# NNU-GISA/MetricSfM

Hardware: AMD Instinct MI355X
Metric: BA iterations/sec (higher is better)
Workload: dtype f64; 1 GPU; BASELINE config 3: 500 cameras / 200000 points / 1200000 observations, dense-Schur LM, Huber(1); reduced_system_order=3003, parallelism=points sharded over 1 rank(s), camera block all-reduced, collective=none (1 rank), successful_steps=2789, unsuccessful_steps=0

## Files before the change

### include/msfm.h

```cpp
#ifndef MSFM_H_
#define MSFM_H_

#include <stddef.h>
#include <stdint.h>

#ifdef __cplusplus
extern "C" {
#endif

#define MSFM_VERSION 100

#define MSFM_OK 0
#define MSFM_E_INVAL (-1)
#define MSFM_E_NOMEM (-2)
#define MSFM_E_DEVICE (-3)
#define MSFM_E_NUMERIC (-4)

typedef struct msfm_ctx msfm_ctx;

int msfm_version(void);
int msfm_ctx_create(int device, msfm_ctx** out);
void msfm_ctx_destroy(msfm_ctx* ctx);
const char* msfm_last_error(const msfm_ctx* ctx);
void* msfm_ctx_stream(msfm_ctx* ctx);
// ... 65 lines not shown

typedef struct msfm_ba_options {
  int max_num_iterations;
  int num_threads;
  int progress_to_stdout;
  double huber_delta;
  double function_tolerance;
  double gradient_tolerance;
  double parameter_tolerance;
  double initial_trust_region_radius;
  double max_trust_region_radius;
  double min_trust_region_radius;
  double min_relative_decrease;
  double min_lm_diagonal;
  double max_lm_diagonal;
  int max_num_consecutive_invalid_steps;
  int jacobi_scaling;
} msfm_ba_options;
void msfm_ba_options_default(msfm_ba_options* opt);

#define MSFM_BA_CONVERGENCE_FUNCTION 1
#define MSFM_BA_CONVERGENCE_GRADIENT 2
#define MSFM_BA_CONVERGENCE_PARAMETER 3
#define MSFM_BA_NO_CONVERGENCE 4
#define MSFM_BA_FAILURE 5
#define MSFM_BA_MIN_RADIUS 6

typedef struct msfm_ba_iteration {
  double cost;
  double cost_change;
  double gradient_max_norm;
  double step_norm;
  double relative_decrease;
  double trust_region_radius;
  int32_t step_is_valid;
  int32_t step_is_successful;
} msfm_ba_iteration;

typedef struct msfm_ba_summary {
  int termination;
  int num_iterations;
  int num_successful_steps;
  int num_unsuccessful_steps;
  double initial_cost, final_cost;
  int num_residuals;
  int num_reduced_params;
  msfm_ba_iteration* iterations;
  int iterations_capacity;
  double solve_ms;
  double setup_ms;
} msfm_ba_summary;

int msfm_ba_solve(msfm_ctx* ctx, msfm_ba_problem* problem, const msfm_ba_options* options,
                  msfm_ba_summary* summary);

typedef struct msfm_ba msfm_ba;
int msfm_ba_create(msfm_ctx* ctx, const msfm_ba_problem* problem, msfm_ba** out);
int msfm_ba_run(msfm_ba* ba, const msfm_ba_options* options, msfm_ba_summary* summary);
int msfm_ba_upload_params(msfm_ba* ba, const double* cam_pose, const double* cam_model,
                          const double* point);
int msfm_ba_download_params(msfm_ba* ba, double* cam_pose, double* cam_model, double* point);
void msfm_ba_destroy(msfm_ba* ba);
typedef struct msfm_ba_layout {
  int reduced_order;
  int system_order;
  int n_domains;
  int domain_cols[8];
  int separator_cols;
  int panel_launches;
  int n_levels;
  int level_nodes[3];
  int level_begin[3];
  int root_cols;
  long long cc_entries, cc_entries_folded;
  int fold_slots, fold_passes;
  long long mc_entries, mc_entries_folded;
  int fold_mc_slots;
  int solve_paths;
  int npb_S, npb_L, npb_X;
  int npb_S4;
  int assemble_paths;
  int rider_paths;
  long long fold_parts, fold_crit_steps, fold_crit_steps_unsplit, fold_wave_steps;
} msfm_ba_layout;
#define MSFM_PATH_ASM_BESIDE 1
#define MSFM_PATH_RIDER_MODELSUM (1 << 8)
#define MSFM_PATH_RIDER_UPDATE (1 << 9)
#define MSFM_PATH_LEVEL_CHAIN(l) (1 << (l))
#define MSFM_PATH_ROOT_CHAIN (1 << 3)
#define MSFM_PATH_BACKSOLVE_CHAIN (1 << 4)
int msfm_ba_get_layout(const msfm_ba* ba, msfm_ba_layout* out);

int msfm_camera_graph_dissection(int n_cams, const uint8_t* adjacency, int tail_cols, int force_depth, int32_t* label,
                                 int* n_leaves, int* chain_steps);

#define MSFM_REDUCE_SUM 0
#define MSFM_REDUCE_MAX 1
typedef int (*msfm_allreduce_fn)(void* user, double* buf_dev, size_t count, int op, void* stream);
int msfm_ctx_set_allreduce(msfm_ctx* ctx, msfm_allreduce_fn fn, void* user, int rank,
                           int world_size);

#define MSFM_RCCL_ID_BYTES 128
int msfm_rccl_get_unique_id(msfm_ctx* ctx, unsigned char id[MSFM_RCCL_ID_BYTES]);
int msfm_ctx_init_rccl(msfm_ctx* ctx, const unsigned char id[MSFM_RCCL_ID_BYTES], int rank, int world_size);
int msfm_ctx_allreduce(msfm_ctx* ctx, double* buf_dev, size_t count, int op);


typedef struct msfm_tracks {
  int n_tracks, n_cams;
  const int32_t* track_off;
  const int32_t* track_cam;
  const double* track_xy;
  const double* cam_R;
  const double* cam_t;
  const double* cam_c;
  const double* cam_fk;
} msfm_tracks;

int msfm_triangulate_midpoint_batch(msfm_ctx* ctx, const msfm_tracks* tracks, double th_error,
                                    double th_angle, double* X, double* mse, uint8_t* ok);
int msfm_triangulate_dlt_batch(msfm_ctx* ctx, const msfm_tracks* tracks, double th_error,
                               double th_angle, double* X, double* mse, uint8_t* ok);
int msfm_reproject_mse_batch(msfm_ctx* ctx, const msfm_tracks* tracks, const double* X,
                             double* mse);

int msfm_epipolar_filter(msfm_ctx* ctx, const float* pt1, const float* pt2, int n,
                         const double F[9], double th, uint8_t* inlier);

typedef struct msfm_fransac_options {
  double threshold;
  double confidence;
  int max_iterations;
  int min_points;
  int min_inliers;
  uint64_t seed;
} msfm_fransac_options;
void msfm_fransac_default_options(msfm_fransac_options* opt);
int msfm_fundamental_ransac_batch(msfm_ctx* ctx, int n_pairs, const int* offsets, const float* pt1,
                                  const float* pt2, const msfm_fransac_options* opt, double* F,
                                  uint8_t* inlier, int* n_inliers, uint8_t* ok);
typedef struct msfm_hransac_options {
  double threshold;
  double confidence;
  int max_iterations;
  int polish;
  uint64_t seed;
} msfm_hransac_options;
void msfm_hransac_default_options(msfm_hransac_options* opt);
int msfm_homography_ransac_batch(msfm_ctx* ctx, int n_pairs, const int* offsets, const float* pt1, const float* pt2,
                                 const msfm_hransac_options* opt, double* H , uint8_t* inlier ,
                                 int* n_inliers, uint8_t* ok);

typedef struct msfm_slam_prior_options {
  int win_size;
  int th_same_pts;
  float th_epipolar;
  float th_distance;
  float th_ratio_f;
  float th_h_f_ratio;
  uint64_t seed_f, seed_h;
} msfm_slam_prior_options;
void msfm_slam_prior_default_options(msfm_slam_prior_options* opt);
int msfm_slam_priors(msfm_ctx* ctx, const msfm_tracks* points, const msfm_slam_prior_options* opt, int* n_pairs,
                     int* pairs, double* F, double* H, int* n_candidates, int* candidates);

int msfm_epipolar_filter_batch(msfm_ctx* ctx, int n_pairs, const int* offsets, const float* pt1,
                               const float* pt2, const double* F, const uint8_t* ok, double th,
// ... 358 lines not shown
```

### metricsfm_amd/_abi.py

```python
import ctypes as C

import numpy as np

c_double_p = C.POINTER(C.c_double)
c_float_p = C.POINTER(C.c_float)
c_int_p = C.POINTER(C.c_int32)
c_u8_p = C.POINTER(C.c_uint8)

MSFM_OK = 0
MSFM_E_INVAL, MSFM_E_NOMEM, MSFM_E_DEVICE, MSFM_E_NUMERIC = -1, -2, -3, -4
MSFM_MATCH_GOOD = 0x40000000
MSFM_MATCH_NOT_ALL = 0x20000000
MSFM_MATCH_ID_MASK = 0x1FFFFFFF
MSFM_MAX_KERNEL_STATS = 32
MSFM_PATH_ROOT_CHAIN = 1 << 3
MSFM_PATH_BACKSOLVE_CHAIN = 1 << 4
MSFM_PATH_ASM_BESIDE = 1
MSFM_PATH_RIDER_MODELSUM = 1 << 8
MSFM_PATH_RIDER_UPDATE = 1 << 9


def MSFM_PATH_LEVEL_CHAIN(level):
    return 1 << level


TERMINATION = {1: "CONVERGENCE_FUNCTION", 2: "CONVERGENCE_GRADIENT", 3: "CONVERGENCE_PARAMETER",
               4: "NO_CONVERGENCE", 5: "FAILURE", 6: "MIN_RADIUS"}


class BaProblem(C.Structure):
    _fields_ = [("n_cams", C.c_int), ("n_models", C.c_int), ("n_points", C.c_int), ("n_obs", C.c_int),
                ("cam_pose", c_double_p), ("cam_model", c_double_p), ("cam_model_of_cam", c_int_p),
                ("point", c_double_p), ("obs_cam", c_int_p), ("obs_pt", c_int_p), ("obs_xy", c_double_p),
                ("pt_weight", c_double_p), ("cam_mutable", c_u8_p), ("model_mutable", c_u8_p),
                ("pt_mutable", c_u8_p), ("gps_xyz", c_double_p), ("gps_weight", C.c_double)]


class BaLayout(C.Structure):
    _fields_ = [("reduced_order", C.c_int), ("system_order", C.c_int), ("n_domains", C.c_int), ("domain_cols", C.c_int * 8),
                ("separator_cols", C.c_int), ("panel_launches", C.c_int), ("n_levels", C.c_int), ("level_nodes", C.c_int * 3),
                ("level_begin", C.c_int * 3), ("root_cols", C.c_int),
                ("cc_entries", C.c_longlong), ("cc_entries_folded", C.c_longlong), ("fold_slots", C.c_int), ("fold_passes", C.c_int),
                ("mc_entries", C.c_longlong), ("mc_entries_folded", C.c_longlong), ("fold_mc_slots", C.c_int), ("solve_paths", C.c_int),
                ("npb_S", C.c_int), ("npb_L", C.c_int), ("npb_X", C.c_int), ("npb_S4", C.c_int), ("assemble_paths", C.c_int),
                ("rider_paths", C.c_int), ("fold_parts", C.c_longlong), ("fold_crit_steps", C.c_longlong),
                ("fold_crit_steps_unsplit", C.c_longlong), ("fold_wave_steps", C.c_longlong)]


class FransacOptions(C.Structure):
    _fields_ = [("threshold", C.c_double), ("confidence", C.c_double), ("max_iterations", C.c_int),
                ("min_points", C.c_int), ("min_inliers", C.c_int), ("seed", C.c_uint64)]


class PairSelectOptions(C.Structure):
    _fields_ = [("th_init_matches", C.c_int32), ("th_inliers", C.c_int32), ("max_hypotheses", C.c_int32), ("fransac", FransacOptions)]


class HransacOptions(C.Structure):
    _fields_ = [("threshold", C.c_double), ("confidence", C.c_double), ("max_iterations", C.c_int), ("polish", C.c_int),
                ("seed", C.c_uint64)]


class SlamPriorOptions(C.Structure):
    _fields_ = [("win_size", C.c_int), ("th_same_pts", C.c_int), ("th_epipolar", C.c_float), ("th_distance", C.c_float),
                ("th_ratio_f", C.c_float), ("th_h_f_ratio", C.c_float), ("seed_f", C.c_uint64), ("seed_h", C.c_uint64)]


class EpnpfOptions(C.Structure):
    _fields_ = [("f_ratio_min", C.c_double), ("f_ratio_max", C.c_double), ("f_ratio_step", C.c_double), ("max_iter", C.c_int32),
                ("seed", C.c_uint64)]


class SlamMatchOptions(C.Structure):
    _fields_ = [("th_first_second_ratio", C.c_float), ("th_epipolar", C.c_float), ("th_distance", C.c_float)]


class BaOptions(C.Structure):
    _fields_ = [("max_num_iterations", C.c_int), ("num_threads", C.c_int), ("progress_to_stdout", C.c_int),
                ("huber_delta", C.c_double), ("function_tolerance", C.c_double),
                ("gradient_tolerance", C.c_double), ("parameter_tolerance", C.c_double),
                ("initial_trust_region_radius", C.c_double), ("max_trust_region_radius", C.c_double),
                ("min_trust_region_radius", C.c_double), ("min_relative_decrease", C.c_double),
                ("min_lm_diagonal", C.c_double), ("max_lm_diagonal", C.c_double),
                ("max_num_consecutive_invalid_steps", C.c_int), ("jacobi_scaling", C.c_int)]


class BaIteration(C.Structure):
    _fields_ = [("cost", C.c_double), ("cost_change", C.c_double), ("gradient_max_norm", C.c_double),
                ("step_norm", C.c_double), ("relative_decrease", C.c_double),
                ("trust_region_radius", C.c_double), ("step_is_valid", C.c_int32),
                ("step_is_successful", C.c_int32)]


class BaSummary(C.Structure):
    _fields_ = [("termination", C.c_int), ("num_iterations", C.c_int), ("num_successful_steps", C.c_int),
                ("num_unsuccessful_steps", C.c_int), ("initial_cost", C.c_double), ("final_cost", C.c_double),
                ("num_residuals", C.c_int), ("num_reduced_params", C.c_int),
                ("iterations", C.POINTER(BaIteration)), ("iterations_capacity", C.c_int),
                ("solve_ms", C.c_double), ("setup_ms", C.c_double)]


class Tracks(C.Structure):
    _fields_ = [("n_tracks", C.c_int), ("n_cams", C.c_int), ("track_off", c_int_p), ("track_cam", c_int_p),
                ("track_xy", c_double_p), ("cam_R", c_double_p), ("cam_t", c_double_p), ("cam_c", c_double_p),
                ("cam_fk", c_double_p)]


class LocalizeProblem(C.Structure):
    _fields_ = [("n_cams", C.c_int32), ("cam_img", c_int_p), ("feat_point", c_int_p), ("n_points", C.c_int32), ("pt_bad", c_u8_p),
                ("pt_mse", c_double_p), ("pt_views", c_int_p), ("n_cand", C.c_int32), ("cand_img", c_int_p), ("fail_times", c_int_p),
                ("point_xyz", c_double_p), ("keypoints", c_float_p)]


class LocalizePoseOptions(C.Structure):
    _fields_ = [("th_mse_localization", C.c_double), ("th_min_2d3d_corres", C.c_int32), ("max_iter", C.c_int32), ("seed", C.c_uint64),
                ("sweep", EpnpfOptions), ("first_row", C.c_int32), ("max_tries", C.c_int32)]


class SeedOptions(C.Structure):
    _fields_ = [("th_mse_reprojection", C.c_double), ("th_angle_small", C.c_double), ("th_seedpair_structures", C.c_int32),
                ("ransac_times_5pt", C.c_int32), ("ransac_times_8pt", C.c_int32), ("seed_5pt", C.c_uint64), ("seed_8pt", C.c_uint64)]


class SeedProblem(C.Structure):
    _fields_ = [("n_hyp", C.c_int32), ("hyp_img", c_int_p), ("cam_fk", c_double_p), ("same_model", c_u8_p), ("keypoints", c_float_p)]


class NewPointsOptions(C.Structure):
    _fields_ = [("th_mse_reprojection", C.c_double), ("th_angle_small", C.c_double), ("th_angle_large", C.c_double),
# ... 125 lines not shown
```

### metricsfm_amd/capi.py

```python
import ctypes as C
import os

import numpy as np

from . import _abi as A
from . import _header
from ._header import ALLREDUCE_FN

_HERE = os.path.dirname(os.path.abspath(__file__))
LIB_PATH = os.environ.get("MSFM_LIB") or os.path.join(_HERE, "libmsfm.so")
_lib = None

with open(_header.HEADER) as _f:
    PROTOTYPES = _header.prototypes(_f.read())
SYMBOLS = list(PROTOTYPES)


class MsfmError(RuntimeError):
    def __init__(self, code, text):
        super().__init__("libmsfm error %d: %s" % (code, text))
        self.code = code


def lib():
# ... 1099 lines not shown
        with _Handle(h, "msfm_round_set_destroy"):
            out = _round_set_result(self.ctx, h, z["n_cams"], z["n_models"], 0, partial, full, o.keep_problem, capacity)
        for k in ("point_xyz", "pt_mutable", "pt_bad", "pt_mse", "pt_new_added", "pt_views"):
            del out[k]
        return out


class LocalizeSet(_Handle):
    _destroy = "msfm_localize_set_destroy"

    def __init__(self, ctx: Context, h):
        self.ctx, self._h = ctx, h
        nk, nc, nv, hp, nb = C.c_int32(), C.c_int32(), C.c_int32(), C.c_int32(), C.c_int64()
        lib().msfm_localize_set_size(h, C.byref(nk), C.byref(nc), C.byref(nv), C.byref(hp), C.byref(nb))
        self.n_kept, self.n_corr, self.n_visible, self.has_points, self.h2d_bytes = nk.value, nc.value, nv.value, bool(hp.value), nb.value

    def fetch(self):
        nk, nc, nv = self.n_kept, self.n_corr, self.n_visible
        rank, coff, voff = np.zeros(max(1, nk), np.int32), np.zeros(nk + 1, np.int32), np.zeros(nk + 1, np.int32)
        cf, cp, vc = np.zeros(max(1, nc), np.int32), np.zeros(max(1, nc), np.int32), np.zeros(max(1, nv), np.int32)
        pw = np.zeros((max(1, nc), 3)) if self.has_points else None
        p2 = np.zeros((max(1, nc), 2)) if self.has_points else None
        lib().msfm_localize_set_fetch(self._h, A.ptr(rank, A.c_int_p), A.ptr(coff, A.c_int_p), A.ptr(cf, A.c_int_p), A.ptr(cp, A.c_int_p),
                                      A.ptr(voff, A.c_int_p), A.ptr(vc, A.c_int_p), A.ptr(pw, A.c_double_p), A.ptr(p2, A.c_double_p))
        out = dict(rank=rank[:nk], corr_off=coff, corr_feat=cf[:nc], corr_point=cp[:nc], vis_off=voff, vis_cam=vc[:nv], h2d_bytes=self.h2d_bytes)
        if self.has_points:
            out["pts_w"], out["pts_2d"] = pw[:nc], p2[:nc]
        return out

    def poses(self, row_f, row_f_init=None, n_points=0, pt_new_added=None, **opts):
        n = self.n_kept
        f = A.as_c(np.broadcast_to(np.asarray(row_f, dtype=np.float64), (n,)).copy(), np.float64)
        fi = None if row_f_init is None else A.as_c(np.broadcast_to(np.asarray(row_f_init, dtype=np.float64), (n,)).copy(), np.float64)
        added = None if pt_new_added is None else A.as_c(np.asarray(pt_new_added, dtype=np.uint8).reshape(-1), np.uint8)
        if added is not None:
            if n_points and n_points != len(added):
                raise ValueError("pt_new_added must hold n_points entries")
            n_points = len(added)
        o = localize_pose_options(**opts)
        h = C.c_void_p()
        self.ctx.check(lib().msfm_localize_poses(self.ctx._h, self._h, A.ptr(f, A.c_double_p), A.ptr(fi, A.c_double_p), int(n_points),
                                                 A.ptr(added, A.c_u8_p), C.byref(o), C.byref(h)))
        with _Handle(h, "msfm_localize_pose_set_destroy"):
            nr, nc, ntr, win, nxt = (C.c_int32() for _ in range(5))
            lib().msfm_localize_pose_set_size(h, C.byref(nr), C.byref(nc), C.byref(ntr), C.byref(win), C.byref(nxt))
            nc, m = nc.value, max(1, n)
            tried, arm, pas, state = np.zeros(m, np.uint8), np.zeros(m, np.uint8), np.zeros(m, np.uint8), np.zeros(max(1, nc), np.uint8)
            fo, R, t, avg, err = np.zeros(m), np.zeros((m, 3, 3)), np.zeros((m, 3)), np.zeros(m), np.zeros(max(1, nc))
            bs, bi, nin, nout = (np.zeros(m, np.int32) for _ in range(4))
            dp, ip, up = A.c_double_p, A.c_int_p, A.c_u8_p
            lib().msfm_localize_pose_set_fetch(h, A.ptr(tried, up), A.ptr(arm, up), A.ptr(pas, up), A.ptr(fo, dp), A.ptr(R, dp), A.ptr(t, dp),
                                               A.ptr(avg, dp), A.ptr(bs, ip), A.ptr(bi, ip), A.ptr(nin, ip), A.ptr(nout, ip), A.ptr(err, dp),
                                               A.ptr(state, up))
        return {"tried": tried[:n], "arm": arm[:n], "pass": pas[:n], "f": fo[:n], "R": R[:n], "t": t[:n], "avg_error": avg[:n],
                "best_step": bs[:n], "best_iter": bi[:n], "n_inliers": nin[:n], "n_outliers": nout[:n], "errors": err[:nc],
                "corr_state": state[:nc], "n_tried": ntr.value, "winner": win.value, "next_row": nxt.value}


class BaResident(_Handle):
    _destroy = "msfm_ba_destroy"

    def __init__(self, ctx: Context, arrays: A.BaArrays):
        self.ctx, self.arrays = ctx, arrays
        self._h = C.c_void_p()
        ctx.check(lib().msfm_ba_create(ctx._h, C.byref(arrays.struct), C.byref(self._h)))

    def run(self, options=None, capacity=512):
        options = options or default_options()
        buf = A.SummaryBuf(capacity)
        self.ctx.check(lib().msfm_ba_run(self._h, C.byref(options), C.byref(buf.struct)))
        return buf.result()

    def layout(self):
        lay = A.BaLayout()
        self.ctx.check(lib().msfm_ba_get_layout(self._h, C.byref(lay)))
        return dict(reduced_order=lay.reduced_order, system_order=lay.system_order, n_domains=lay.n_domains,
                    domain_cols=list(lay.domain_cols)[:max(0, lay.n_domains if lay.n_domains > 1 else 0)],
                    separator_cols=lay.separator_cols, panel_launches=lay.panel_launches, n_levels=lay.n_levels,
                    level_nodes=list(lay.level_nodes)[:lay.n_levels], level_begin=list(lay.level_begin)[:lay.n_levels], root_cols=lay.root_cols,
                    fold=dict(cc_entries=lay.cc_entries, cc_entries_folded=lay.cc_entries_folded, slots=lay.fold_slots, passes=lay.fold_passes,
                              mc_entries=lay.mc_entries, mc_entries_folded=lay.mc_entries_folded, mc_slots=lay.fold_mc_slots,
                              parts=lay.fold_parts, crit_steps=lay.fold_crit_steps, crit_steps_unsplit=lay.fold_crit_steps_unsplit,
                              wave_steps=lay.fold_wave_steps),
                    solve_paths=lay.solve_paths, assemble_paths=lay.assemble_paths, rider_paths=lay.rider_paths, npb_S=lay.npb_S, npb_L=lay.npb_L, npb_X=lay.npb_X, npb_S4=lay.npb_S4)

    def upload(self, cam_pose=None, cam_model=None, point=None):
        cp, cm, pt = A.as_c(cam_pose, np.float64), A.as_c(cam_model, np.float64), A.as_c(point, np.float64)
        self.ctx.check(lib().msfm_ba_upload_params(self._h, A.ptr(cp, A.c_double_p), A.ptr(cm, A.c_double_p),
                                                   A.ptr(pt, A.c_double_p)))

    def download(self):
        a = self.arrays
        cp, cm, pt = np.zeros_like(a.cam_pose), np.zeros_like(a.cam_model), np.zeros_like(a.point)
        self.ctx.check(lib().msfm_ba_download_params(self._h, A.ptr(cp, A.c_double_p), A.ptr(cm, A.c_double_p),
                                                     A.ptr(pt, A.c_double_p)))
        return cp, cm, pt


class MultiContext(_Handle):
    _destroy = "msfm_multi_destroy"

    def __init__(self, n_gpus, devices=None):
        self._h = C.c_void_p()
        dev = None if devices is None else A.as_c(np.asarray(devices, dtype=np.int32), np.int32)
        rc = lib().msfm_ctx_create_multi(n_gpus, None if dev is None else A.ptr(dev, A.c_int_p), C.byref(self._h))
        if rc != 0:
            raise MsfmError(rc, "msfm_ctx_create_multi failed")
        self.n = lib().msfm_multi_size(self._h)

    def check(self, rc):
        if rc != 0:
            raise MsfmError(rc, lib().msfm_multi_last_error(self._h).decode())

    def ba_solve(self, arrays: A.BaArrays, options=None, capacity=512):
        options = options or default_options()
        buf = A.SummaryBuf(capacity)
        self.check(lib().msfm_multi_ba_solve(self._h, C.byref(arrays.struct), C.byref(options), C.byref(buf.struct)))
        return buf.result()

    def _tri(self, fn, tracks, th_error, th_angle):
        n = tracks.struct.n_tracks
        X, mse, ok = np.zeros((n, 3)), np.zeros(n), np.zeros(n, dtype=np.uint8)
        self.check(fn(self._h, C.byref(tracks.struct), th_error, th_angle, A.ptr(X, A.c_double_p), A.ptr(mse, A.c_double_p), A.ptr(ok, A.c_u8_p)))
        return X, mse, ok

    def triangulate_midpoint(self, tracks, th_error, th_angle):
        return self._tri(lib().msfm_multi_triangulate_midpoint_batch, tracks, th_error, th_angle)

    def triangulate_dlt(self, tracks, th_error, th_angle):
        return self._tri(lib().msfm_multi_triangulate_dlt_batch, tracks, th_error, th_angle)

    def reproject_mse(self, tracks, X):
        X = A.as_c(X, np.float64)
        mse = np.zeros(tracks.struct.n_tracks)
        self.check(lib().msfm_multi_reproject_mse_batch(self._h, C.byref(tracks.struct), A.ptr(X, A.c_double_p), A.ptr(mse, A.c_double_p)))
        return mse

    def match_pairs(self, descs, pairs, ratio_good=0.6, ratio_all=0.85):
        descs = [A.as_c(d, np.float32) for d in descs]
        pairs = A.as_c(np.asarray(pairs, dtype=np.int32).reshape(-1, 2), np.int32)
        count = np.array([len(d) for d in descs], dtype=np.int32)
        dp = (A.c_float_p * len(descs))(*[A.ptr(d, A.c_float_p) if len(d) else None for d in descs])
        codes = [np.zeros(max(1, int(count[j])), np.int32) for _, j in pairs]
        cp = (A.c_int_p * max(1, len(pairs)))(*[A.ptr(c, A.c_int_p) for c in codes])
        na, ng = np.zeros(max(1, len(pairs)), np.int32), np.zeros(max(1, len(pairs)), np.int32)
        self.check(lib().msfm_multi_match_pairs(self._h, len(descs), dp, A.ptr(count, A.c_int_p), 128, A.ptr(pairs, A.c_int_p), len(pairs),
                                                ratio_good, ratio_all, cp, A.ptr(na, A.c_int_p), A.ptr(ng, A.c_int_p)))
        return [c[:count[j]] for c, (_, j) in zip(codes, pairs)], na[:len(pairs)], ng[:len(pairs)]


def camera_graph_dissection(adjacency, tail_cols=4, force_depth=-1):
    adj = np.ascontiguousarray(adjacency, dtype=np.uint8)
    n = adj.shape[0]
    assert adj.shape == (n, n)
    label = np.zeros(n, np.int32)
    nl, steps = C.c_int(0), C.c_int(0)
    rc = lib().msfm_camera_graph_dissection(n, A.ptr(adj, A.c_u8_p), int(tail_cols), int(force_depth), A.ptr(label, A.c_int_p), C.byref(nl),
                                            C.byref(steps))
    if rc != 0:
        raise MsfmError(rc, "msfm_camera_graph_dissection")
    return label, nl.value, steps.value
```

### metricsfm_amd/csrc/ba.hip

```cpp
#include <algorithm>
#include <array>
#include <chrono>
#include <cmath>
#include <cstdlib>
#include <cstring>
#include <functional>

#include <rocprim/rocprim.hpp>

#include "ba_device.h"
#include "ba_partials.h"
#include "common.h"
#include "solve_riders.h"


#define PSTRIDE 80
#define CHUNK 1024
#define FTF_CHUNK 512
static int chunk_for(long total, int max_chunk) {
  const long c = 64 * ((total / 1024 + 63) / 64);
  return (int)std::max<long>(64, std::min<long>(max_chunk, c));
}
#define F_JCJC 0
#define F_JMJC 36
// ... 137 lines not shown
}
template <bool WRITE_JAC>
__global__ __launch_bounds__(256) void k_gps(int ncb, const int* __restrict__ cb_cam, const double* __restrict__ cam,
                                              const double* __restrict__ gps, double w, double huber,
                                              const double* __restrict__ scale_c, double* __restrict__ g_r,
                                              double* __restrict__ g_J, double* __restrict__ cost_partial, const double* __restrict__ spec = nullptr) {
  __shared__ double sh[4];
  if (spec && spec[0] == 0.0) return;
  gps_block<WRITE_JAC>(blockIdx.x, ncb, cb_cam, cam, gps, w, huber, scale_c, g_r, g_J, cost_partial, sh);
}

struct ReduceJobs {
  int count;
  struct { const double* p; int n; int slot; int is_max; } job[6];
  const int* fail;
  int fail_slot;
};
__global__ __launch_bounds__(1024) void k_reduce(ReduceJobs J, double* __restrict__ scal) {
  __shared__ double sh[16];
  const double* __restrict__ partial = J.job[blockIdx.x].p;
  const int n = J.job[blockIdx.x].n, slot = J.job[blockIdx.x].slot, is_max = J.job[blockIdx.x].is_max;
  double v0 = 0.0, v1 = 0.0, v2 = 0.0, v3 = 0.0;
  int i = threadIdx.x;
  for (; i + 3072 < n; i += 4096) {
    const double a = partial[i], b = partial[i + 1024], c = partial[i + 2048], d = partial[i + 3072];
    if (is_max) { v0 = fmax(v0, a); v1 = fmax(v1, b); v2 = fmax(v2, c); v3 = fmax(v3, d); }
    else { v0 += a; v1 += b; v2 += c; v3 += d; }
  }
  for (; i < n; i += 1024) v0 = is_max ? fmax(v0, partial[i]) : v0 + partial[i];
  double v = is_max ? fmax(fmax(v0, v1), fmax(v2, v3)) : (v0 + v1) + (v2 + v3);
  v = is_max ? wave_max(v) : wave_sum(v);
  if ((threadIdx.x & 63) == 0) sh[threadIdx.x >> 6] = v;
  __syncthreads();
  if (threadIdx.x == 0) {
    double t = sh[0];
    for (int w = 1; w < 16; w++) t = is_max ? fmax(t, sh[w]) : t + sh[w];
    scal[slot] = t;
    if (blockIdx.x == 0 && J.fail) scal[J.fail_slot] = (double)*J.fail;
  }
}

struct FoldPass { int off, words, quad0, n_quads, n_diag, flip, pad1, pad2; };
#define FOLD_HDR_IDLE (1u << 10)
__host__ __device__ inline unsigned fold_hdr(int first, int count, int part, int parts) {
  return (unsigned)first | ((unsigned)part << 10) | ((unsigned)(parts - 1) << 12) | ((unsigned)count << 16);
}
__host__ __device__ inline int fold_hdr_first(unsigned h) { return (int)(h & 0x3ffu); }
__host__ __device__ inline int fold_hdr_part(unsigned h) { return (int)(h >> 10) & 3; }
__host__ __device__ inline int fold_hdr_parts(unsigned h) { return ((int)(h >> 12) & 3) + 1; }
__host__ __device__ inline int fold_hdr_count(unsigned h) { return (int)(h >> 16); }
#define FOLD_PART_CAP 8
__host__ __device__ inline int fold_parts(int count) { return count <= FOLD_PART_CAP ? 1 : count > 3 * FOLD_PART_CAP ? 4 : (count + FOLD_PART_CAP - 1) / FOLD_PART_CAP; }
__host__ __device__ inline int fold_part_len(int count, int parts, int k) {
  if (count > 4 * FOLD_PART_CAP) return count / parts + (k < count % parts ? 1 : 0);
  return k + 1 < parts ? FOLD_PART_CAP : count - (parts - 1) * FOLD_PART_CAP;
}
struct PointPtrs {
  BaPtrs B;
  PtMap map;
  int npb, NCR;
  const int *pt_first, *pm_first, *pm_mb;
  double *diag_p;
  double *ptL, *ptg, *T, *Tu, *Tm, *Tmu;
  double radius, dmin, dmax;
  int reuse_diag, mode;
  int store_rows;
  double* cost_partial;
  int* fail;
  const int *fold_wg, *fold_wg_pass_first, *fold_slot_rank;
  const FoldPass* fold_pass;
  const unsigned* fold_stream;
  double* fold_partial;
  double* fold_mc_partial;
  const double* spec;
};

#define GROUP_SUM4(x) { x += dpp_f64<MSFM_DPP_XOR1>(x); x += dpp_f64<MSFM_DPP_XOR2>(x); }
#define GROUP_SUM(x) { if constexpr (LPP == 16) x += dpp_f64<MSFM_DPP_ROR8>(x); GROUP_SUM4(x) if constexpr (LPP != 4) x += dpp_f64<MSFM_DPP_HALF_MIRROR>(x); }

#define FOLD_NREC 256
#define FOLD_WORDS 1024
#define FOLD_PASS_SLOTS 128
#define FOLD_PASS_QUADS 256
template <int LPP>
__device__ __forceinline__ void k_point_body(const PointPtrs& P, double* __restrict__ gmax_partial, double* sh, double* park, unsigned* ent_s) {
  constexpr int GW = LPP ? LPP : 8;
  constexpr bool single = LPP != 0;
  const int tid = threadIdx.x, sub = tid & (GW - 1);
  const int pb = ptmap_wg_first(P.map, blockIdx.x) + tid / GW;
  const bool act = pb < ptmap_wg_end(P.map, blockIdx.x);
  const bool fold = single && P.fold_wg != nullptr && P.mode != 1 && P.fold_wg[blockIdx.x] != 0;
  const int wv = __builtin_amdgcn_readfirstlane(tid >> 6);
  auto stage = [&](int off, int words) {
    if (256 * wv < words)
      __builtin_amdgcn_global_load_lds((const __attribute__((address_space(1))) void*)(P.fold_stream + (size_t)off + 256 * wv + 4 * (tid & 63)),
                                       (__attribute__((address_space(3))) void*)(ent_s + 256 * wv), 16, 0, 0);
  };
  int fp0 = 0, fp1 = 0;
  if (fold) {
    fp0 = __builtin_amdgcn_readfirstlane(P.fold_wg_pass_first[blockIdx.x]);
    fp1 = __builtin_amdgcn_readfirstlane(P.fold_wg_pass_first[blockIdx.x + 1]);
    stage(__builtin_amdgcn_readfirstlane(P.fold_pass[fp0].off), __builtin_amdgcn_readfirstlane(P.fold_pass[fp0].words));
  }
  int f = 0, l = 0;
  if (act) { f = P.pt_first[pb]; l = P.pt_first[pb + 1]; }
  double V00 = 0, V10 = 0, V11 = 0, V20 = 0, V21 = 0, V22 = 0, g0 = 0, g1 = 0, g2 = 0;
  double cost = 0.0;
  auto lin_row = [&](int i) {
    double r0, r1, jcs[12], jms[6], jps[6];
    const double ci = obs_linearize(P.B, i, r0, r1, jcs, jms, jps);
    if constexpr (single) {
#pragma unroll
      for (int k = 0; k < 12; k++) park[k * 256 + tid] = jcs[k];
#pragma unroll
      for (int k = 0; k < 6; k++) { park[(12 + k) * 256 + tid] = jms[k]; park[(18 + k) * 256 + tid] = jps[k]; }
    }
    if (P.store_rows) cost += ci;
    const double a0 = jps[0], a1 = jps[1], a2 = jps[2], b0 = jps[3], b1 = jps[4], b2 = jps[5];
    V00 += a0 * a0 + b0 * b0; V10 += a1 * a0 + b1 * b0; V11 += a1 * a1 + b1 * b1;
    V20 += a2 * a0 + b2 * b0; V21 += a2 * a1 + b2 * b1; V22 += a2 * a2 + b2 * b2;
    g0 += a0 * r0 + b0 * r1; g1 += a1 * r0 + b1 * r1; g2 += a2 * r0 + b2 * r1;
  };
  if constexpr (single) {
    if (f + sub < l) lin_row(f + sub);
  } else {
    for (int base = f; base < l; base += 8)
      if (base + sub < l) lin_row(base + sub);
  }
  GROUP_SUM(V00) GROUP_SUM(V10) GROUP_SUM(V11) GROUP_SUM(V20) GROUP_SUM(V21) GROUP_SUM(V22)
  GROUP_SUM(g0) GROUP_SUM(g1) GROUP_SUM(g2)

  double gmax = 0.0;
  double l00 = 1, l10 = 0, l11 = 1, l20 = 0, l21 = 0, l22 = 1, i00 = 1, i11 = 1, i22 = 1, u0 = 0, u1 = 0, u2 = 0;
  if (act) {
    double* dg = P.diag_p + 3 * (size_t)pb;
    if (P.mode == 1) {
      if (sub == 0) { dg[0] = V00; dg[1] = V11; dg[2] = V22; }
    } else {
      double d0, d1, d2;
      if (!P.reuse_diag) {
        d0 = fmin(fmax(V00, P.dmin), P.dmax); d1 = fmin(fmax(V11, P.dmin), P.dmax); d2 = fmin(fmax(V22, P.dmin), P.dmax);
        if (sub == 0) { dg[0] = d0; dg[1] = d1; dg[2] = d2; }
      } else {
        d0 = dg[0]; d1 = dg[1]; d2 = dg[2];
      }
      const double radius = P.spec ? P.spec[1] : P.radius;
      const double q0 = sqrt(d0 / radius), q1 = sqrt(d1 / radius), q2 = sqrt(d2 / radius);
      V00 += q0 * q0; V11 += q1 * q1; V22 += q2 * q2;
      bool ok = V00 > 0.0;
      l00 = sqrt(V00);
      l10 = V10 / l00; l20 = V20 / l00;
      const double e1 = V11 - l10 * l10;
      ok = ok && e1 > 0.0;
      l11 = sqrt(e1);
      l21 = (V21 - l20 * l10) / l11;
      const double e2 = V22 - l20 * l20 - l21 * l21;
      ok = ok && e2 > 0.0;
      l22 = sqrt(e2);
      i00 = 1.0 / l00; i11 = 1.0 / l11; i22 = 1.0 / l22;
      u0 = g0 * i00;
      u1 = (g1 - l10 * u0) * i11;
      u2 = (g2 - l20 * u0 - l21 * u1) * i22;
      if (sub == 0) {
        if (!ok) atomicOr(P.fail, 2);
        double* L = P.ptL + 6 * (size_t)pb;
        L[0] = i00; L[1] = l10; L[2] = i11; L[3] = l20; L[4] = l21; L[5] = i22;
        const double* sp = P.B.scale_p + 3 * (size_t)pb;
        gmax = fmax(fabs(g0 / sp[0]), fmax(fabs(g1 / sp[1]), fabs(g2 / sp[2])));
      }
    }
  }
  if (P.mode != 1) {
    const int wl = tid & 63, tsrc = GW == 16 ? ((wl & 3) << 4) | (wl >> 2) : GW == 4 ? ((wl & 15) << 2) | (wl >> 4) : ((wl & 7) << 3) | (wl >> 3);
    const bool need_T = !fold || P.fold_mc_partial == nullptr;
    auto round = [&](int rd, double (&Tk)[18], int& cpk) {
      const int i = f + rd + sub;
      int cp = -1;
      if (i < l) cp = P.B.o_cpos[i];
      double T[18], tu[6];
#pragma unroll
      for (int k = 0; k < 18; k++) T[k] = 0.0;
#pragma unroll
      for (int k = 0; k < 6; k++) tu[k] = 0.0;
      if (cp >= 0) {
        double jcs[12], jms[6], jps[6];
        if (!single) { double r0, r1; obs_linearize(P.B, i, r0, r1, jcs, jms, jps); }
        else {
#pragma unroll
          for (int k = 0; k < 12; k++) jcs[k] = park[k * 256 + tid];
#pragma unroll
          for (int k = 0; k < 6; k++) jps[k] = park[(18 + k) * 256 + tid];
        }
        const double a0 = jps[0], a1 = jps[1], a2 = jps[2], b0 = jps[3], b1 = jps[4], b2 = jps[5];
#pragma unroll
        for (int a = 0; a < 6; a++) {
          const double ja = jcs[a], jb = jcs[6 + a];
          const double w0 = ja * a0 + jb * b0, w1 = ja * a1 + jb * b1, w2 = ja * a2 + jb * b2;
          const double t0 = w0 * i00;
          const double t1 = (w1 - l10 * t0) * i11;
          const double t2 = (w2 - l20 * t0 - l21 * t1) * i22;
          T[a * 3 + 0] = t0; T[a * 3 + 1] = t1; T[a * 3 + 2] = t2;
          tu[a] = t0 * u0 + t1 * u1 + t2 * u2;
        }
      }
      cpk = cp;
#pragma unroll
      for (int k = 0; k < 18; k++) Tk[k] = T[k];
      if (!need_T) {
        if (cp >= 0) {
          double2* Tu2 = reinterpret_cast<double2*>(P.Tu + 6 * (size_t)cp);
#pragma unroll
          for (int k = 0; k < 3; k++) Tu2[k] = make_double2(tu[2 * k], tu[2 * k + 1]);
        }
        return;
      }
      const int cpt = __shfl(cp, tsrc, 64);
      if (need_T) {
#pragma unroll
        for (int k = 0; k < 18; k++) T[k] = __shfl(T[k], tsrc, 64);
      }
#pragma unroll
      for (int k = 0; k < 6; k++) tu[k] = __shfl(tu[k], tsrc, 64);
      if (cpt >= 0) {
        double2* Tu2 = reinterpret_cast<double2*>(P.Tu + 6 * (size_t)cpt);
#pragma unroll
        for (int k = 0; k < 3; k++) Tu2[k] = make_double2(tu[2 * k], tu[2 * k + 1]);
        if (need_T) {
#pragma unroll
          for (int k = 0; k < 18; k++) P.T[(size_t)k * P.NCR + cpt] = T[k];
        }
      }
    };
    double* const H0 = park;
    double* const H1 = park + FOLD_NREC * 10;
    double* const TM4 = park + 2 * FOLD_NREC * 10;
    auto tm_slot = [&](int rec0, int k) -> double* {
      if constexpr (LPP == 4) return TM4 + (rec0 >> 2) * 9 + k;
      else return ((k & 1) ? H1 : H0) + (rec0 + (k >> 1)) * 10 + 9;
    };
    auto rec_st = [&](int rec, const double (&Tk)[18]) {
#pragma unroll
      for (int k = 0; k < 9; k++) { H0[rec * 10 + k] = Tk[k]; H1[rec * 10 + k] = Tk[9 + k]; }
    };
    {
      double Tk[18];
      int cpk;
      round(0, Tk, cpk);
      int pe0 = 0, pe1 = 0, my_mb = -2;
      if (act) {
        pe0 = P.pm_first[pb]; pe1 = P.pm_first[pb + 1];
        if (f + sub < l) my_mb = P.B.o_mb[f + sub];
      }
      double pjm[6], pjp[6];
      if constexpr (single) {
#pragma unroll
// ... 86 lines not shown
          const int sl = 64 * rd + ((rd & 1) ? sl4 ^ flip : sl4);
          const bool on = sl < n_quads;
          const unsigned h = on ? ent_s[sl] : FOLD_HDR_IDLE;
          const int part = fold_hdr_part(h), n_parts = fold_hdr_parts(h);
          const int e0 = hdr + fold_hdr_first(h), e1 = e0 + fold_hdr_count(h);
          int rnk = 0;
          if (on && part == 0) rnk = P.fold_slot_rank[quad0 + sl];
          const bool mcd = sl < n_diag;
          const int ma0 = ra ? 2 : 0;
          double acc[9], accm[6];
#pragma unroll
          for (int k = 0; k < 9; k++) acc[k] = 0.0;
#pragma unroll
          for (int k = 0; k < 6; k++) accm[k] = 0.0;
          for (int e = e0; e < e1; e++) {
            const unsigned pr = ent_s[e];
            const double* oi = (ra ? H1 : H0) + (int)(pr & 0xffffu) * 10;
            const double* oj = (rb ? H1 : H0) + (int)(pr >> 16) * 10;
            double ti[9], tj[9];
#pragma unroll
            for (int k2 = 0; k2 < 4; k2++) {
              const double2 vi = *reinterpret_cast<const double2*>(oi + 2 * k2);
              const double2 vj = *reinterpret_cast<const double2*>(oj + 2 * k2);
              ti[2 * k2] = vi.x; ti[2 * k2 + 1] = vi.y; tj[2 * k2] = vj.x; tj[2 * k2 + 1] = vj.y;
            }
            ti[8] = oi[8]; tj[8] = oj[8];
#pragma unroll
            for (int a = 0; a < 3; a++)
#pragma unroll
              for (int c = 0; c < 3; c++)
                acc[a * 3 + c] += ti[a * 3] * tj[c * 3] + ti[a * 3 + 1] * tj[c * 3 + 1] + ti[a * 3 + 2] * tj[c * 3 + 2];
            if (mcd && (pr & 0xffffu) == (pr >> 16)) {
              const int r0 = (int)(pr & 0xffffu) & ~(GW - 1);
              double tm[6];
#pragma unroll
              for (int k6 = 0; k6 < 6; k6++) { const int k = 3 * ma0 + k6; tm[k6] = *tm_slot(r0, k); }
#pragma unroll
              for (int a = 0; a < 2; a++)
#pragma unroll
                for (int c = 0; c < 3; c++)
                  accm[a * 3 + c] += tm[a * 3] * tj[c * 3] + tm[a * 3 + 1] * tj[c * 3 + 1] + tm[a * 3 + 2] * tj[c * 3 + 2];
            }
          }
          if (__any(n_parts > 1)) {
            const bool pair = (part & 1) == 0 && part + 1 < n_parts, last = part == 0 && n_parts > 2;
            auto gather = [&](double& v) {
              const double up1 = dpp_f64<MSFM_DPP_SHL4>(v);
              if (pair) v += up1;
              const double up2 = dpp_f64<MSFM_DPP_SHL8>(v);
              if (last) v += up2;
            };
#pragma unroll
            for (int k = 0; k < 9; k++) gather(acc[k]);
#pragma unroll
            for (int k = 0; k < 6; k++) gather(accm[k]);
          }
          if (on && part == 0) {
            if (mcd) {
              double* om = P.fold_mc_partial + (size_t)rnk * 18;
#pragma unroll
              for (int a = 0; a < 2; a++)
                if (ma0 + a < 3) {
#pragma unroll
                  for (int c = 0; c < 3; c++) om[(ma0 + a) * 6 + 3 * rb + c] = accm[a * 3 + c];
                }
            }
            double* out = P.fold_partial + (size_t)rnk * 36;
#pragma unroll
            for (int a = 0; a < 3; a++)
#pragma unroll
              for (int c = 0; c < 3; c++) out[(3 * ra + a) * 6 + 3 * rb + c] = acc[a * 3 + c];
          }
        }
      }
    }
  }
  if (P.store_rows) {
    const double tc = block_sum256(cost, sh);
    if (threadIdx.x == 0) P.cost_partial[blockIdx.x] = tc;
  }
  const double t = block_max256(gmax, sh);
  if (threadIdx.x == 0) gmax_partial[blockIdx.x] = t;
}
__global__ __launch_bounds__(256) __attribute__((amdgpu_waves_per_eu(3, 3))) void k_point(PointPtrs P, double* __restrict__ gmax_partial) {
  __shared__ double sh[4];
  __shared__ double park[24 * 256];
  __shared__ __attribute__((aligned(16))) unsigned ent_s[FOLD_WORDS];
  if (P.spec && P.spec[0] == 0.0) return;
  const int lanes = ptmap_lanes(P.map, blockIdx.x);
  if (lanes == 4) k_point_body<4>(P, gmax_partial, sh, park, ent_s);
  else if (lanes == 8) k_point_body<8>(P, gmax_partial, sh, park, ent_s);
  else if (lanes == 16) k_point_body<16>(P, gmax_partial, sh, park, ent_s);
  else k_point_body<0>(P, gmax_partial, sh, park, ent_s);
}

__global__ __launch_bounds__(256) void k_cam_rows(int A, const int* __restrict__ o_cpos, const int* __restrict__ o_pt, const double* __restrict__ o_x,
                                                   const double* __restrict__ o_y, const double* __restrict__ o_w, int* __restrict__ cm_pt,
                                                   double* __restrict__ cm_x, double* __restrict__ cm_y, double* __restrict__ cm_w, int* __restrict__ cm_row) {
  const int i = blockIdx.x * 256 + threadIdx.x;
  if (i >= A) return;
  const int cp = o_cpos[i];
  if (cp < 0) return;
  cm_pt[cp] = o_pt[i]; cm_x[cp] = o_x[i]; cm_y[cp] = o_y[i]; cm_w[cp] = o_w[i]; cm_row[cp] = i;
}
__global__ __launch_bounds__(256) void k_cam_points(int ncr, const int* __restrict__ cm_pt, const double* __restrict__ pt, double* __restrict__ X0,
                                                     double* __restrict__ X1) {
  const int e = blockIdx.x * 256 + threadIdx.x;
  if (e >= ncr) return;
  const size_t p = (size_t)cm_pt[e];
#pragma unroll
  for (int j = 0; j < 3; j++) { const double v = pt[3 * p + j]; X0[3 * (size_t)e + j] = v; X1[3 * (size_t)e + j] = v; }
}
__global__ __launch_bounds__(256) void k_chunk_cam(int nchunk, const int* __restrict__ ch_start, const int* __restrict__ cm_row, const int* __restrict__ o_cam,
                                                    const int* __restrict__ o_model, const int* __restrict__ o_cb, const int* __restrict__ o_mb,
                                                    int4* __restrict__ chunk_cam) {
  const int ch = blockIdx.x * 256 + threadIdx.x;
  if (ch >= nchunk) return;
  const int i = cm_row[ch_start[ch]];
  chunk_cam[ch] = make_int4(o_cam[i], o_model[i], o_cb[i], o_mb[i]);
}

template <int N>
__device__ __forceinline__ void wave_reduce_store(double (&acc)[N], double* out, int lane) {
  double v;
  int k;
  wave_reduce_scatter<N>(acc, lane, v, k);
  if (k >= 0) out[k] = v;
}

struct CamRows {
  const int* pt;
  const double* X;
  const double *x, *y, *w;
  const int4* chunk_cam;
};
__device__ __forceinline__ void ftf_body(int blk, int nchunk, const int* __restrict__ ch_start, const int* __restrict__ ch_end, const BaPtrs& P, const CamRows& R,
                                         const double* __restrict__ Tu, const int* __restrict__ cpos_pb, double* __restrict__ partial) {
  const int chunk = blk * 4 + (threadIdx.x >> 6), lane = threadIdx.x & 63;
  if (chunk >= nchunk) return;
  constexpr int O_JC = 0, O_JMC = 21, O_JM = 39, O_CR = 45, O_MR = 51, O_TU = 54;
  double acc[60];
#pragma unroll
  for (int k = 0; k < 60; k++) acc[k] = 0.0;
  const int4 cc = R.chunk_cam[chunk];
  const int c = __builtin_amdgcn_readfirstlane(cc.x), m = __builtin_amdgcn_readfirstlane(cc.y);
  const int cb = __builtin_amdgcn_readfirstlane(cc.z), mb = __builtin_amdgcn_readfirstlane(cc.w);
  double pose[6], rc[4], cm[3], sc[6], sm[3];
  const double sp[3] = {0.0, 0.0, 0.0};
#pragma unroll
  for (int j = 0; j < 6; j++) { pose[j] = P.cam[6 * (size_t)c + j]; sc[j] = cb >= 0 ? P.scale_c[6 * cb + j] : 0.0; }
#pragma unroll
  for (int j = 0; j < 4; j++) rc[j] = P.rot[4 * (size_t)c + j];
#pragma unroll
  for (int j = 0; j < 3; j++) { cm[j] = P.model[3 * (size_t)m + j]; sm[j] = mb >= 0 ? P.scale_m[3 * mb + j] : 0.0; }
  const int e1 = ch_end[chunk];
  int e = ch_start[chunk] + lane;
  double xn = 0, yn = 0, wn = 0, Xn[3] = {0, 0, 0};
  if (e < e1) {
    xn = R.x[e]; yn = R.y[e]; wn = R.w[e];
#pragma unroll
    for (int j = 0; j < 3; j++) Xn[j] = R.X[3 * (size_t)e + j];
  }
  for (; e < e1; e += 64) {
    const double X[3] = {Xn[0], Xn[1], Xn[2]};
    const double ox = xn, oy = yn, ow = wn;
    const bool has_tu = cpos_pb[e] >= 0;
    double2 tu2[3];
    if (has_tu) {
      const double2* tp = reinterpret_cast<const double2*>(Tu + 6 * (size_t)e);
#pragma unroll
      for (int a = 0; a < 3; a++) tu2[a] = tp[a];
    }
    if (e + 64 < e1) {
      xn = R.x[e + 64]; yn = R.y[e + 64]; wn = R.w[e + 64];
#pragma unroll
      for (int j = 0; j < 3; j++) Xn[j] = R.X[3 * (size_t)(e + 64) + j];
// ... 69 lines not shown
}
__global__ __launch_bounds__(128) void k_camftf(int ncb, const int* __restrict__ cam_chunk_first,
                                                 const double* __restrict__ partial, double* __restrict__ camftf,
                                                 const double* __restrict__ g_r, const double* __restrict__ g_J, int add_gps, int post,
                                                 double* __restrict__ diag_c, const double* __restrict__ scale_c, int reuse_diag, int mode,
                                                 double dmin, double dmax, double* __restrict__ gmax_c, CamFinish fin) {
  __shared__ double sums[PSTRIDE];
  const int cb = blockIdx.x, t = threadIdx.x;
  if (cb >= ncb) {
    const int i = (cb - ncb) * 128 + t;
    if (i < fin.n_padcol) fin.M[(size_t)fin.padcol[i] * fin.ld + fin.padcol[i]] = 1.0;
    return;
  }
  if (t < PSTRIDE) {
    double s = 0.0;
    int ch = cam_chunk_first[cb];
    const int ch1 = cam_chunk_first[cb + 1];
    for (; ch + 4 <= ch1; ch += 4) {
      const double* q = partial + (size_t)ch * PSTRIDE + t;
      const double p0 = q[0], p1 = q[PSTRIDE], p2 = q[2 * PSTRIDE], p3 = q[3 * PSTRIDE];
      s += p0; s += p1; s += p2; s += p3;
    }
    for (; ch < ch1; ch++) s += partial[(size_t)ch * PSTRIDE + t];
    if (add_gps) {
      if (t >= F_JCJC && t < F_JCJC + 36) {
        const int a = (t - F_JCJC) / 6, b = (t - F_JCJC) % 6;
        if (a == b && a >= 3) { const double j = g_J[3 * (size_t)cb + a - 3]; s += j * j; }
      } else if (t >= F_JCR + 3 && t < F_JCR + 6) {
        const int k = t - F_JCR - 3;
        s += g_J[3 * (size_t)cb + k] * g_r[3 * (size_t)cb + k];
      }
    }
    camftf[(size_t)cb * PSTRIDE + t] = s;
    sums[t] = s;
  }
  if (!post) return;
  __syncthreads();
  if (t < 6) {
    const int i = 6 * cb + t;
    const double d = sums[F_JCJC + t * 6 + t];
    if (mode == 1) diag_c[i] = d;
    else if (!reuse_diag) diag_c[i] = fmin(fmax(d, dmin), dmax);
    gmax_c[i] = fabs(sums[F_JCR + t] / scale_c[i]);
  }
  if (!fin.M) return;
  __syncthreads();
  const int off = fin.cb_off[cb];
  if (t < 18) {
    const int e = 2 * t, a = e / 6, c = e % 6;
    double2* at = reinterpret_cast<double2*>(&fin.M[(size_t)(off + a) * fin.ld + off + c]);
    double2 v = *at;
    cc_diag_finish(v.x, v.y, sums[F_JCJC + e], sums[F_JCJC + e + 1], a, c, diag_c + 6 * (size_t)cb, fin.radius);
    *at = v;
  } else if (t >= 32 && t < 50) {
    const int e = t - 32, mb = fin.cb_mb[cb];
    if (mb >= 0) fin.M[(size_t)(fin.mo + 3 * mb + e / 6) * fin.ld + off + e % 6] += sums[F_JMJC + e];
  } else if (t >= 64 && t < 70) {
    const int a = t - 64;
    fin.M[(size_t)fin.n * fin.ld + off + a] = sums[F_JCR + a] - sums[F_TU + a];
  }
}

__global__ void k_cam_post(int ncb, const double* __restrict__ camftf, double* __restrict__ diag_c,
                           const double* __restrict__ scale_c, int reuse_diag, int mode, double dmin, double dmax,
                           double* __restrict__ gmax_c) {
  const int i = blockIdx.x * blockDim.x + threadIdx.x;
  if (i >= 6 * ncb) return;
  const int cb = i / 6, a = i % 6;
  const double* f = camftf + (size_t)cb * PSTRIDE;
  const double s = f[F_JCJC + a * 6 + a];
  if (mode == 1) diag_c[i] = s;
  else if (!reuse_diag) diag_c[i] = fmin(fmax(s, dmin), dmax);
  gmax_c[i] = fabs(f[F_JCR + a] / scale_c[i]);
}

__global__ __launch_bounds__(128) void k_modelsum(ModelSumArgs A) {
  __shared__ double mmacc[13];
  modelsum_body(A, blockIdx.x, threadIdx.x, mmacc);
}

__global__ void k_make_scale(int n, const double* __restrict__ norm2, double* __restrict__ scale) {
  const int i = blockIdx.x * blockDim.x + threadIdx.x;
  if (i < n) scale[i] = 1.0 / (1.0 + sqrt(norm2[i]));
}

template <int DA, int DB, bool WITH_U, bool SPARSE = false>
__device__ __forceinline__ void pairs_body(int blk, int nblk, int nchunk, const int* __restrict__ ch_start, const int* __restrict__ ch_end,
                                           const int* __restrict__ pa, const int* __restrict__ pb,
                                           const double* __restrict__ TA, const double* __restrict__ TB,
                                           const double* __restrict__ UA, size_t plane, double* __restrict__ partial,
                                           const int* __restrict__ live) {
  constexpr int NOUT = DA * DB + (WITH_U ? DA : 0);
  const int nwg = nblk, xcd = blk & 7, loc = blk >> 3;
  const int qn = nwg >> 3, rm = nwg & 7;
  const int swz = (xcd < rm ? xcd * (qn + 1) : rm * (qn + 1) + (xcd - rm) * qn) + loc;
  const int cidx = swz * 4 + (threadIdx.x >> 6), lane = threadIdx.x & 63;
  if (cidx >= nchunk) return;
  const int chunk = live ? live[cidx] : cidx;
  double acc[NOUT];
#pragma unroll
  for (int k = 0; k < NOUT; k++) acc[k] = 0.0;
  const int e0 = ch_start[chunk] + lane, e1 = ch_end[chunk];
  constexpr int NPRE = SPARSE ? CHUNK / 64 : 1;
  int pre_a[NPRE];
  if constexpr (SPARSE) {
#pragma unroll
    for (int k = 0; k < NPRE; k++) pre_a[k] = e0 + 64 * k < e1 ? pa[e0 + 64 * k] : -1;
  }
#pragma unroll 1
  for (int e = e0, step = 0; e < e1 || (SPARSE && step < NPRE); e += 64, step++) {
    int ia;
    if constexpr (SPARSE) {
      if (step >= NPRE) break;
      ia = -1;
#pragma unroll
      for (int k = 0; k < NPRE; k++) if (k == step) ia = pre_a[k];
      if (__builtin_amdgcn_ballot_w64(ia >= 0) == 0ull) continue;
    } else {
      ia = pa[e];
    }
    if (ia < 0) continue;
    const int ib = pb[e];
    double ta[DA * 3], tb[DB * 3];
    if constexpr (DA == 6) {
#pragma unroll
      for (int k = 0; k < 18; k++) ta[k] = TA[(size_t)k * plane + ia];
    } else {
      const double* pa_ = TA + (size_t)ia * (DA * 3);
#pragma unroll
      for (int k = 0; k < DA * 3; k++) ta[k] = pa_[k];
    }
    if constexpr (DB == 6) {
#pragma unroll
      for (int k = 0; k < 18; k++) tb[k] = TB[(size_t)k * plane + ib];
    } else {
      const double* pb_ = TB + (size_t)ib * (DB * 3);
#pragma unroll
      for (int k = 0; k < DB * 3; k++) tb[k] = pb_[k];
    }
#pragma unroll
    for (int a = 0; a < DA; a++)
#pragma unroll
      for (int b = 0; b < DB; b++)
        acc[a * DB + b] += ta[a * 3] * tb[b * 3] + ta[a * 3 + 1] * tb[b * 3 + 1] + ta[a * 3 + 2] * tb[b * 3 + 2];
    if (WITH_U && ia == ib) {
#pragma unroll
      for (int a = 0; a < DA; a++) acc[DA * DB + a] += UA[(size_t)ia * DA + a];
    }
  }
  wave_reduce_store<NOUT>(acc, partial + (size_t)chunk * NOUT, lane);
}
template <int DA, int DB, bool WITH_U>
__global__ __launch_bounds__(256) void k_pairs(int nchunk, const int* __restrict__ ch_start, const int* __restrict__ ch_end,
                                                const int* __restrict__ pa, const int* __restrict__ pb,
                                                const double* __restrict__ TA, const double* __restrict__ TB,
                                                const double* __restrict__ UA, size_t plane, double* __restrict__ partial) {
  pairs_body<DA, DB, WITH_U>(blockIdx.x, gridDim.x, nchunk, ch_start, ch_end, pa, pb, TA, TB, UA, plane, partial, nullptr);
}

struct ZeroMap { unsigned char lev[256]; short lo[256], hi[256]; int nb; };
__device__ __forceinline__ void zero_tile_body(int tile, double* __restrict__ M, int ld, const ZeroMap& Z) {
  int I = (int)((sqrt(8.0 * tile + 1.0) - 1.0) * 0.5);
  while (I * (I + 1) / 2 > tile) I--;
  while ((I + 1) * (I + 2) / 2 <= tile) I++;
  const int J = tile - I * (I + 1) / 2;
  const bool same = Z.lev[I] == Z.lev[J] && Z.lo[I] == Z.lo[J] && Z.hi[I] == Z.hi[J];
// ... 491 lines not shown
      for (int j = 0; j < 3; j++) { const double sj = -z[6 * ncb + 3 * mb + j]; m0 += lin_Jm[(size_t)j * As + it] * sj; m1 += lin_Jm[(size_t)(3 + j) * As + it] * sj; }
    mcc -= m0 * (lin_r[it] + m0 / 2.0) + m1 * (lin_r[As + it] + m1 / 2.0);
  } else if (has_gps && t < nrest + ncb) {
    const int cb = t - nrest;
    for (int k = 0; k < 3; k++) {
      const double m = g_J[3 * (size_t)cb + k] * (-z[6 * cb + 3 + k]);
      mcc -= m * (g_r[3 * (size_t)cb + k] + m / 2.0);
    }
  }
  const double s = block_sum256(mcc, sh);
  if (threadIdx.x == 0) mcc_partial[blk] = s;
}

struct TailArgs {
  int n_zero; double* M; int ld; ZeroMap Z;
  int n_mcc, n_cost, n_gps;
  int A, AE, ncb; const int *o_cb, *o_mb; const double *lin_r, *lin_Jc, *lin_Jm, *z; int has_gps; const double *g_r, *g_J; double* mcc_partial;
  BaPtrs P; double* cost_partial;
  const int* cb_cam; const double *cam_c, *gps; double gps_weight, huber; const double* scale_c; double *g_r_w, *g_J_w;
};
__global__ __launch_bounds__(256) void k_tail(TailArgs a) {
  __shared__ double sh[4];
  int b = blockIdx.x;
  if (b < a.n_zero) { zero_tile_body(b, a.M, a.ld, a.Z); return; }
  b -= a.n_zero;
  if (b < a.n_mcc) { mcc_rest_block(b, a.A, a.AE, a.ncb, a.o_cb, a.o_mb, a.lin_r, a.lin_Jc, a.lin_Jm, a.z, a.has_gps, a.g_r, a.g_J, a.mcc_partial, sh); return; }
  b -= a.n_mcc;
  if (b < a.n_cost) { linearize_block<false>(a.P, 0, b, a.cost_partial, sh); return; }
  b -= a.n_cost;
  gps_block<false>(b, a.ncb, a.cb_cam, a.cam_c, a.gps, a.gps_weight, a.huber, a.scale_c, a.g_r_w, a.g_J_w, a.cost_partial + a.n_cost, sh);
}

__global__ void k_zero_int(int* p) { *p = 0; }
enum { LM_NONE = 0, LM_INVALID, LM_PARAM_TOL, LM_FUNC_TOL, LM_ACCEPT, LM_REJECT };
enum { H_SEQ = 16, H_CODE = 17, H_RADIUS = 18 };
struct LmDecide {
  int on;
  int fresh;
  double x_cost, radius;
  double min_relative_decrease, parameter_tolerance, function_tolerance, max_radius, min_radius;
};
__device__ __forceinline__ double cube_rn(double t) {
  const double h = t * t, l = fma(t, t, -h);
  const double p = h * t, e = fma(h, t, -p);
  return p + fma(l, t, e);
}
__global__ __launch_bounds__(64) void k_publish_scalars(const double* __restrict__ scal, double* h_scal, unsigned long long seq, int* fail, LmDecide D,
                                                        double* __restrict__ spec) {
  const int lane = threadIdx.x;
  if (lane < 16) __hip_atomic_store(&h_scal[lane], scal[lane], __ATOMIC_RELAXED, __HIP_MEMORY_SCOPE_SYSTEM);
  if (lane == 0) {
    int code = LM_NONE;
    double rnew = D.radius;
    if (D.on) {
      const double mcc = scal[S_MCC], cand = scal[S_COST], dx2 = scal[S_DX2], x2 = scal[S_X2];
      const double xc = D.fresh ? scal[S_XCOST] : D.x_cost;
      const bool solved = (int)scal[S_FAIL] == 0;
      if (!(solved && mcc > 0.0)) code = LM_INVALID;
      else if (sqrt(dx2) <= D.parameter_tolerance * (sqrt(x2) + D.parameter_tolerance)) code = LM_PARAM_TOL;
      else if (fabs(xc - cand) <= D.function_tolerance * xc) code = LM_FUNC_TOL;
      else {
        const double rho = (xc - cand) / mcc;
        if (rho > D.min_relative_decrease) {
          code = LM_ACCEPT;
          rnew = D.radius / fmax(1.0 / 3.0, 1.0 - cube_rn(2.0 * rho - 1.0));
          rnew = fmin(D.max_radius, rnew);
        } else code = LM_REJECT;
      }
    }
    spec[0] = (code == LM_ACCEPT && rnew > D.min_radius) ? 1.0 : 0.0;
    spec[1] = rnew;
    __hip_atomic_store(&h_scal[H_CODE], (double)code, __ATOMIC_RELAXED, __HIP_MEMORY_SCOPE_SYSTEM);
    __hip_atomic_store(&h_scal[H_RADIUS], rnew, __ATOMIC_RELAXED, __HIP_MEMORY_SCOPE_SYSTEM);
  }
  __threadfence_system();
  if (lane == 0) {
    __hip_atomic_store(reinterpret_cast<unsigned long long*>(h_scal + H_SEQ), seq, __ATOMIC_RELEASE, __HIP_MEMORY_SCOPE_SYSTEM);
    if (fail) *fail = 0;
  }
}
__global__ void k_fill(int n, double v, double* __restrict__ p) {
  const int i = blockIdx.x * 256 + threadIdx.x;
  if (i < n) p[i] = v;
}

template <bool PACK>
__global__ __launch_bounds__(256) void k_pack_blocks(int nblk, const int* __restrict__ u_row, const int* __restrict__ u_col,
                                                      const int* __restrict__ cb_off, double* __restrict__ M, int ld,
                                                      double* __restrict__ pack) {
  const int e = blockIdx.x * 256 + threadIdx.x;
  if (e >= nblk * 36) return;
  const int b = e / 36, t = e - 36 * b;
  const size_t at = (size_t)(cb_off[u_row[b]] + t / 6) * ld + cb_off[u_col[b]] + t % 6;
  if (PACK) pack[e] = M[at];
  else M[at] = pack[e];
}

struct FoldTables {
  bool on = false;
  bool all = false;
  int n_live = 0;
  DevBuf<int> live_chunk;
  int n_wg = 0, n_slots = 0, n_entries = 0, n_pass = 0;
  long long n_parts = 0, crit_steps = 0, crit_steps_unsplit = 0, wave_steps = 0;
  DevBuf<int> wg_fold, wg_pass_first, slot_rank, blk_range;
  DevBuf<uint8_t> blk_live;
  DevBuf<FoldPass> pass;
  DevBuf<unsigned> stream;
  DevBuf<double> partial;
  bool mc_on = false, mc_all = false;
  int n_diag = 0, mc_n_live = 0;
  long long mc_entries_folded = 0;
  DevBuf<int> mc_range, mc_live_chunk;
  DevBuf<double> mc_partial;
};

struct PairJobs {
  int n_pairs = 0, n_chunks = 0, n_blocks = 0;
  DevBuf<int> pa, pb, ch_start, ch_end, blk_row, blk_col, blk_chunk_first;
  DevBuf<double> partial;
  std::vector<int> h_row, h_col;
};

struct msfm_ba {
  msfm_ctx* ctx = nullptr;
  msfm_env env;
  int world_at_create = 1;
  double setup_ms = 0;
  int Nc = 0, Nm = 0, Np = 0;
  int ncb = 0, nmb = 0, npb = 0, nred = 0, npad = 0;
  PtMap map = {0, 0, 0, 0, 0, 0, 0};
  int n_short4 = 0;
  int nsys = 0, mo = 0, n_padcol = 0;
  msfm_chol_plan plan;
  int A = 0, AE = 0, NCR = 0, NPM = 0;
  bool has_gps = false;
  double gps_weight = 0;
  int n_residuals = 0;
  std::vector<int> h_cb_cam, h_mb_model, h_pb_pt;
  int n_fchunks = 0;
  int nblk_obs = 0, nblk_pt = 0;
  BaPartials parts;
  int n_ublk = 0;
  bool spec_on = true;
  double* swrite = nullptr;
  msfm_chol_ws* chol_ws = nullptr;
  DevBuf<int> cb_off, padcol;
  DevBuf<double> zsys, corners;
  DevBuf<double> cam, model, pt, cam_c, model_c, pt_c;
  DevBuf<int> cb_cam, mb_model, pb_pt, cb_mb;
  DevBuf<int> o_cam, o_model, o_pt, o_cb, o_mb, o_pb, o_cpos, o_pm;
  DevBuf<double> o_x, o_y, o_w;
  DevBuf<double> lin_r, lin_Jc, lin_Jm, T, Tu, Tm, Tmu, rot, rot_c;
  DevBuf<int> cm_pt;
  DevBuf<double> cm_xyw;
  DevBuf<double> cm_X, cm_Xc;
  DevBuf<int4> chunk_cam;
  DevBuf<int> cpos_pb;
  DevBuf<double> scale_c, scale_m, scale_p, diag_c, diag_m, diag_p;
  DevBuf<int> pt_first, pm_first, pm_mb;
  DevBuf<double> ptL, ptg;
  DevBuf<int> f_start, f_end, cam_chunk_first;
  DevBuf<double> f_partial, camftf, modelsum;
  DevBuf<int> mcam_first, mcam;
  PairJobs cc, mc, mm;
  FoldTables fold;
  DevBuf<double> M, Linv, w, z;
  DevBuf<double> gps, g_r, g_J;
  DevBuf<double> partial, partial2, partial3, partial4, gmax_buf, scal, sloc;
  DevBuf<double> partial_x;
  DevBuf<int> col_param, col_slot;
  DevBuf<double> upd_dx2, upd_x2;
  DevBuf<int> fail;
  double* h_scal = nullptr;
  DevBuf<double> spec;
  double* h_scal_dev = nullptr;
  int* h_fail = nullptr;
  DevBuf<int> u_row, u_col;
  DevBuf<double> pack;
  int zflip = 0;
  unsigned long long scal_seq = 0;
  int solve_paths = 0;
  int asm_paths = 0;
  int rider_paths = 0;
};

struct CamGraph {
  int n = 0;
  std::vector<std::vector<int>> adj;
};

static void graph_levels(const CamGraph& G, const std::vector<char>& in, int start, std::vector<int>& lev) {
  std::fill(lev.begin(), lev.end(), -1);
  std::vector<int> q{start}, nq;
  lev[start] = 0;
  while (!q.empty()) {
    nq.clear();
    for (int u : q)
      for (int v : G.adj[u])
        if (in[v] && lev[v] < 0) { lev[v] = lev[u] + 1; nq.push_back(v); }
    q.swap(nq);
  }
}

static void boundary_cover(const CamGraph& G, const std::vector<int>& L, const std::vector<int>& R, const std::vector<int>& r_index ,
                           std::vector<int>& cover) {
  const int nl = (int)L.size(), nr = (int)R.size();
  std::vector<std::vector<int>> e(nl);
  for (int l = 0; l < nl; l++)
    for (int v : G.adj[L[l]]) if (r_index[v] >= 0) e[l].push_back(r_index[v]);
  std::vector<int> ml(nl, -1), mr(nr, -1), seen(nr, -1), par(nr, -1);
  for (int l = 0; l < nl; l++)
    for (int r : e[l]) if (mr[r] < 0) { mr[r] = l; ml[l] = r; break; }
  std::vector<std::pair<int, size_t>> st;
  int stamp = 0;
  for (int l0 = 0; l0 < nl; l0++) {
    if (ml[l0] >= 0) continue;
    st.clear();
    st.push_back({l0, 0});
    int end = -1;
    while (!st.empty() && end < 0) {
      auto& top = st.back();
      const int l = top.first;
      if (top.second == e[l].size()) { st.pop_back(); continue; }
      const int r = e[l][top.second++];
      if (seen[r] == stamp) continue;
      seen[r] = stamp;
      par[r] = l;
      if (mr[r] < 0) end = r; else st.push_back({mr[r], 0});
    }
    if (end >= 0) stamp++;
    while (end >= 0) { const int l = par[end], prev = ml[l]; ml[l] = end; mr[end] = l; end = prev; }
  }
  std::vector<char> zl(nl, 0), zr(nr, 0);
  std::vector<int> q;
  for (int l = 0; l < nl; l++) if (ml[l] < 0) { zl[l] = 1; q.push_back(l); }
  while (!q.empty()) {
    const int l = q.back();
    q.pop_back();
    for (int r : e[l]) {
      if (zr[r]) continue;
      zr[r] = 1;
      const int l2 = mr[r];
      if (l2 >= 0 && !zl[l2]) { zl[l2] = 1; q.push_back(l2); }
    }
  }
  cover.clear();
  for (int l = 0; l < nl; l++) if (!zl[l]) cover.push_back(L[l]);
  for (int r = 0; r < nr; r++) if (zr[r]) cover.push_back(R[r]);
}

static long steps64(double cams, int tail = 0) { return cdiv(6 * (long)std::ceil(cams) + tail, 64); }
static double chain_estimate(double k, int d, double ns, double total) {
  if (d <= 0) return (double)steps64(k);
  const double s = ns * std::sqrt(std::max(k, 1.0) / std::max(total, 1.0));
  return chain_estimate(std::max((k - s) / 2, 1.0), d - 1, s, k) + (double)steps64(s) + 3;
}

struct CutPrep {
  std::vector<char> in;
  int kind = 0;
  std::vector<char> a, b;
  std::vector<int> order, pos, lo, hi;
  struct Cand { int na, nb, nsep; std::vector<signed char> lab; };
  std::vector<Cand> cands;
  bool cands_done = false;
};
// ... 254 lines not shown
        while (col % 64) padcol_h.push_back(col++);
        L.node[L.K++] = msfm_chol_node{begin, col, node.leaf_lo, node.leaf_hi};
      }
      L.b0 = col;
      if (L.K > 0) nl++;
    }
    ba->plan.n_levels = nl;
    for (int g : T.seps[0][0].cams) place(g);
    if (msfm_env_process().verbose && ctx->rank == 0) {
      fprintf(stderr, "msfm: camera graph %d nodes ->", ng);
      for (int l = 0; l < nl; l++) {
        fprintf(stderr, " level %d:", l);
        for (int k = 0; k < ba->plan.level[l].K; k++) fprintf(stderr, " %d", (ba->plan.level[l].node[k].end - ba->plan.level[l].node[k].begin) / 6);
        fprintf(stderr, " |");
      }
      fprintf(stderr, " root separator %zu cameras\n", T.seps[0][0].cams.size());
    }
  }
  ba->mo = col;
  ba->nsys = col + 3 * ba->nmb;
  ba->n_padcol = (int)padcol_h.size();
}


static int finish_jobs(msfm_ba* ba, PairJobs& J, const std::vector<int>& pa, const std::vector<int>& pb,
                       const std::vector<long>& key_first , const std::vector<int>& brow,
                       const std::vector<int>& bcol, int nout) {
  hipStream_t s = ba->ctx->stream;
  J.n_pairs = (int)pa.size();
  J.n_blocks = (int)brow.size();
  J.h_row = brow;
  J.h_col = bcol;
  std::vector<int> cs, ce, bcf(J.n_blocks + 1, 0);
  const int chunk = chunk_for((long)pa.size(), CHUNK);
  for (int b = 0; b < J.n_blocks; b++) {
    bcf[b] = (int)cs.size();
    for (long e = key_first[b]; e < key_first[b + 1]; e += chunk) {
      cs.push_back((int)e);
      ce.push_back((int)std::min<long>(e + chunk, key_first[b + 1]));
    }
  }
  bcf[J.n_blocks] = (int)cs.size();
  J.n_chunks = (int)cs.size();
  HIP_TRY(ba->ctx, J.pa.from(pa, s));
  HIP_TRY(ba->ctx, J.pb.from(pb, s));
  HIP_TRY(ba->ctx, J.ch_start.from(cs, s));
  HIP_TRY(ba->ctx, J.ch_end.from(ce, s));
  HIP_TRY(ba->ctx, J.blk_row.from(brow, s));
  HIP_TRY(ba->ctx, J.blk_col.from(bcol, s));
  HIP_TRY(ba->ctx, J.blk_chunk_first.from(bcf, s));
  HIP_TRY(ba->ctx, J.partial.alloc((size_t)std::max(1, J.n_chunks) * nout));
  HIP_TRY(ba->ctx, hipStreamSynchronize(s));
  return MSFM_OK;
}

MSFM_API void msfm_ba_options_default(msfm_ba_options* o) {
  if (!o) return;
  o->max_num_iterations = 200;
  o->num_threads = 1;
  o->progress_to_stdout = 0;
  o->huber_delta = 1.0;
  o->function_tolerance = 1e-6;
  o->gradient_tolerance = 1e-10;
  o->parameter_tolerance = 1e-8;
  o->initial_trust_region_radius = 1e4;
  o->max_trust_region_radius = 1e16;
  o->min_trust_region_radius = 1e-32;
  o->min_relative_decrease = 1e-3;
  o->min_lm_diagonal = 1e-6;
  o->max_lm_diagonal = 1e32;
  o->max_num_consecutive_invalid_steps = 5;
  o->jacobi_scaling = 1;
}

MSFM_API void msfm_ba_destroy(msfm_ba* ba) {
  if (!ba) return;
  msfm_ctx* ctx = ba->ctx;
  (void)hipSetDevice(ctx->device);
  (void)hipStreamSynchronize(ctx->stream);
  msfm_chol_ws_destroy(ba->chol_ws);
  ba->chol_ws = nullptr;
  if (ba->h_scal) (void)hipHostFree(ba->h_scal);
  if (ba->h_fail) (void)hipHostFree(ba->h_fail);
  delete ba;
  msfm_ctx_child_released(ctx);
}

struct BaScratch {
  std::vector<int> o_cam, o_model, o_pt, o_cb, o_mb, o_pb, o_cpos, o_pm, run_first, pt_first, cpos_pb, cpos_cb, pa, pb;
  std::vector<double> o_x, o_y, o_w;
  std::vector<std::pair<uint64_t, int>> keyed;
};
static BaScratch& ba_scratch(msfm_ctx* ctx) {
  if (!ctx->ba_scratch) {
    ctx->ba_scratch = new BaScratch();
    ctx->ba_scratch_free = [](void* p) { delete static_cast<BaScratch*>(p); };
  }
  return *static_cast<BaScratch*>(ctx->ba_scratch);
}

namespace devsetup {

template <class T>
__global__ __launch_bounds__(1024) void k_scan_small(const T* __restrict__ in, T* __restrict__ out, int n) {
  __shared__ T part[1024];
  const int t = threadIdx.x, per = (n + 1023) / 1024, lo = min(n, t * per), hi = min(n, lo + per);
  T sum = T(0);
  for (int i = lo; i < hi; i++) sum += in[i];
  part[t] = sum;
  __syncthreads();
  for (int off = 1; off < 1024; off <<= 1) {
    const T v = t >= off ? part[t - off] : T(0);
    __syncthreads();
    part[t] += v;
    __syncthreads();
  }
  T run = part[t] - sum;
  for (int i = lo; i < hi; i++) { const T v = in[i]; out[i] = run; run += v; }
}
#define MSFM_SCAN_SMALL_MAX 65536
template <class T>
static hipError_t excl_scan(const T* in, T* out, size_t n, hipStream_t s, DevBuf<char>& tmp) {
  if (n == 0) return hipSuccess;
  if (n <= MSFM_SCAN_SMALL_MAX && in != out) {
    hipLaunchKernelGGL((k_scan_small<T>), dim3(1), dim3(1024), 0, s, in, out, (int)n);
    return hipGetLastError();
  }
  size_t bytes = 0;
  hipError_t e = rocprim::exclusive_scan(nullptr, bytes, in, out, T(0), n, rocprim::plus<T>(), s);
  if (e != hipSuccess) return e;
  if (tmp.n < bytes) { e = tmp.alloc(bytes); if (e != hipSuccess) return e; }
  return rocprim::exclusive_scan(tmp.p, bytes, in, out, T(0), n, rocprim::plus<T>(), s);
}
template <class K>
static hipError_t sort_pairs(const K* kin, K* kout, const int* vin, int* vout, size_t n, int bits, hipStream_t s, DevBuf<char>& tmp) {
  if (n == 0) return hipSuccess;
  size_t bytes = 0;
  hipError_t e = rocprim::radix_sort_pairs(nullptr, bytes, kin, kout, vin, vout, n, 0, bits, s);
  if (e != hipSuccess) return e;
  if (tmp.n < bytes) { e = tmp.alloc(bytes); if (e != hipSuccess) return e; }
  return rocprim::radix_sort_pairs(tmp.p, bytes, kin, kout, vin, vout, n, 0, bits, s);
}
static int bits_for(long n) { int b = 1; while ((1L << b) < n) b++; return b; }

__device__ __forceinline__ bool dmut(const uint8_t* m, int i) { return m == nullptr || m[i] != 0; }

__global__ __launch_bounds__(256) void k_scan_obs(int No, int Nc, int Np, const int* __restrict__ obs_cam, const int* __restrict__ obs_pt,
                                                   const int* __restrict__ model_of_cam, const uint8_t* __restrict__ cam_mut,
                                                   const uint8_t* __restrict__ model_mut, const uint8_t* __restrict__ pt_mut,
                                                   uint8_t* __restrict__ cu, uint8_t* __restrict__ mu, uint8_t* __restrict__ pu,
                                                   int* __restrict__ cnt, int* __restrict__ err) {
  const int o = blockIdx.x * 256 + threadIdx.x;
  if (o >= No) return;
  const int c = obs_cam[o], p = obs_pt[o];
  if (c < 0 || c >= Nc || p < 0 || p >= Np) { atomicMin(&err[0], o); return; }
  if (o > 0 && p < obs_pt[o - 1]) atomicMin(&err[1], o);
  atomicAdd(&cnt[p], 1);
  const bool cm = dmut(cam_mut, c), pm = dmut(pt_mut, p);
  if (!cm && !pm) return;
  if (pm) pu[p] = 1;
  if (cm) {
    cu[c] = 1;
    const int m = model_of_cam[c];
    if (dmut(model_mut, m)) mu[m] = 1;
  }
}
// ... 1455 lines not shown
  {
    const void* must[] = {ba->cam.p, ba->model.p, ba->pt.p, ba->cam_c.p, ba->model_c.p, ba->pt_c.p, ba->lin_r.p, ba->lin_Jc.p,
                          ba->lin_Jm.p, ba->cm_pt.p, ba->cm_xyw.p, ba->chunk_cam.p, ba->T.p, ba->Tu.p, ba->Tm.p, ba->Tmu.p, ba->scale_c.p,
                          ba->scale_m.p, ba->scale_p.p, ba->diag_c.p, ba->diag_m.p, ba->diag_p.p, ba->ptL.p, ba->ptg.p,
                          ba->f_partial.p, ba->camftf.p, ba->modelsum.p, ba->M.p, ba->Linv.p, ba->w.p, ba->z.p, ba->g_r.p,
                          ba->g_J.p, ba->partial.p, ba->partial2.p, ba->partial3.p, ba->gmax_buf.p, ba->scal.p, ba->fail.p};
    for (const void* q : must)
      if (!q) return msfm_set_error(ctx, MSFM_E_NOMEM, "msfm_ba_create: a device buffer was not allocated");
  }
  lap("allocations");
  ba->swrite = ctx->world > 1 ? ba->sloc.p : ba->scal.p;
  HIP_TRY(ctx, hipMemsetAsync(ba->scal.p, 0, sizeof(double) * S_N, s));
  HIP_TRY(ctx, hipMemsetAsync(ba->sloc.p, 0, sizeof(double) * S_N, s));
  HIP_TRY(ctx, hipHostMalloc((void**)&ba->h_scal, 24 * sizeof(double), hipHostMallocMapped));
  memset(ba->h_scal, 0, 24 * sizeof(double));
  HIP_TRY(ctx, hipHostGetDevicePointer((void**)&ba->h_scal_dev, ba->h_scal, 0));
  HIP_TRY(ctx, hipHostMalloc((void**)&ba->h_fail, 4 * sizeof(int)));
  HIP_TRY(ctx, hipMemsetAsync(ba->z.p, 0, sizeof(double) * (size_t)(ba->npad + 8), s));
  {
    DevBuf<int> cm_row;
    DevScope blk(ctx);
    HIP_TRY(ctx, cm_row.alloc((size_t)std::max(1, NCR)));
    HIP_TRY(ctx, hipMemsetAsync(ba->cm_pt.p, 0, sizeof(int) * (size_t)std::max(1, NCR), s));
    HIP_TRY(ctx, hipMemsetAsync(ba->cm_xyw.p, 0, sizeof(double) * 3 * (size_t)std::max(1, NCR), s));
    HIP_TRY(ctx, hipMemsetAsync(cm_row.p, 0, sizeof(int) * (size_t)std::max(1, NCR), s));
    const size_t ncr = (size_t)std::max(1, NCR);
    if (A > 0)
      hipLaunchKernelGGL(k_cam_rows, dim3(cdiv(A, 256)), dim3(256), 0, s, A, ba->o_cpos.p, ba->o_pt.p, ba->o_x.p, ba->o_y.p, ba->o_w.p, ba->cm_pt.p,
                         ba->cm_xyw.p, ba->cm_xyw.p + ncr, ba->cm_xyw.p + 2 * ncr, cm_row.p);
    if (ba->n_fchunks)
      hipLaunchKernelGGL(k_chunk_cam, dim3(cdiv(ba->n_fchunks, 256)), dim3(256), 0, s, ba->n_fchunks, ba->f_start.p, cm_row.p, ba->o_cam.p, ba->o_model.p,
                         ba->o_cb.p, ba->o_mb.p, ba->chunk_cam.p);
    HIP_TRY(ctx, blk.finish());
  }
  HIP_TRY(ctx, hipMemsetAsync(ba->T.p, 0, sizeof(double) * std::max<size_t>(1, 18 * (size_t)NCR), s));
  HIP_TRY(ctx, hipMemsetAsync(ba->Tu.p, 0, sizeof(double) * std::max<size_t>(1, 6 * (size_t)NCR), s));
  HIP_TRY(ctx, hipMemcpyAsync(ba->cam.p, P->cam_pose, sizeof(double) * 6 * (size_t)Nc, hipMemcpyHostToDevice, s));
  HIP_TRY(ctx, hipMemcpyAsync(ba->model.p, P->cam_model, sizeof(double) * 3 * (size_t)Nm, hipMemcpyHostToDevice, s));
  if (Np) HIP_TRY(ctx, hipMemcpyAsync(ba->pt.p, P->point, sizeof(double) * 3 * (size_t)Np, bulk_on_device ? hipMemcpyDeviceToDevice : hipMemcpyHostToDevice, s));
  HIP_TRY(ctx, hipStreamSynchronize(s));
  lap("done");
  ba->setup_ms = std::chrono::duration<double, std::milli>(std::chrono::steady_clock::now() - t0).count();
  guard.p = nullptr;
  *out = ba;
  return MSFM_OK;
}

MSFM_API int msfm_ba_get_layout(const msfm_ba* ba, msfm_ba_layout* out) {
  if (!ba || !out) return MSFM_E_INVAL;
  memset(out, 0, sizeof *out);
  out->reduced_order = ba->nred;
  out->system_order = ba->nsys;
  const msfm_chol_plan& pl = ba->plan;
  const int K = pl.n_levels > 0 ? pl.level[0].K : 0;
  out->n_domains = K ? K : 1;
  int launches = 0;
  for (int k = 0; k < K; k++) out->domain_cols[k] = pl.level[0].node[k].end - pl.level[0].node[k].begin;
  for (int l = 0; l < pl.n_levels; l++) {
    int maxp = 0;
    for (int k = 0; k < pl.level[l].K; k++) maxp = std::max(maxp, (pl.level[l].node[k].end - pl.level[l].node[k].begin) / 64);
    launches += maxp + 1;
    out->level_nodes[l] = pl.level[l].K;
    out->level_begin[l] = pl.level[l].begin;
  }
  out->n_levels = pl.n_levels;
  const int root_begin = pl.n_levels > 0 ? pl.level[pl.n_levels - 1].b0 : 0;
  out->root_cols = ba->nsys - root_begin;
  out->separator_cols = K ? ba->nsys - pl.level[0].b0 : ba->nsys;
  out->panel_launches = launches + cdiv(out->root_cols, 64);
  if (!K) out->domain_cols[0] = 0;
  out->cc_entries = ba->cc.n_pairs;
  out->mc_entries = ba->mc.n_pairs;
  if (ba->fold.on) {
    out->cc_entries_folded = ba->fold.n_entries;
    out->fold_slots = ba->fold.n_slots;
    out->fold_passes = ba->fold.n_pass;
    out->fold_parts = ba->fold.n_parts; out->fold_crit_steps = ba->fold.crit_steps;
    out->fold_crit_steps_unsplit = ba->fold.crit_steps_unsplit; out->fold_wave_steps = ba->fold.wave_steps;
    if (ba->fold.mc_on) { out->mc_entries_folded = ba->fold.mc_entries_folded; out->fold_mc_slots = ba->fold.n_diag; }
  }
  out->solve_paths = ba->solve_paths;
  out->assemble_paths = ba->asm_paths;
  out->rider_paths = ba->rider_paths;
  out->npb_S = ba->map.nQ + ba->map.nS; out->npb_L = ba->map.nL; out->npb_X = ba->map.nX; out->npb_S4 = ba->n_short4;
  return MSFM_OK;
}

MSFM_API int msfm_ba_upload_params(msfm_ba* ba, const double* cam_pose, const double* cam_model, const double* point) {
  if (!ba) return MSFM_E_INVAL;
  msfm_ctx* ctx = ba->ctx;
  hipStream_t s = ctx->stream;
  if (cam_pose) HIP_TRY(ctx, hipMemcpyAsync(ba->cam.p, cam_pose, sizeof(double) * 6 * (size_t)ba->Nc, hipMemcpyHostToDevice, s));
  if (cam_model) HIP_TRY(ctx, hipMemcpyAsync(ba->model.p, cam_model, sizeof(double) * 3 * (size_t)ba->Nm, hipMemcpyHostToDevice, s));
  if (point && ba->Np) HIP_TRY(ctx, hipMemcpyAsync(ba->pt.p, point, sizeof(double) * 3 * (size_t)ba->Np, hipMemcpyHostToDevice, s));
  HIP_TRY(ctx, hipStreamSynchronize(s));
  return MSFM_OK;
}

MSFM_API int msfm_ba_download_params(msfm_ba* ba, double* cam_pose, double* cam_model, double* point) {
  if (!ba) return MSFM_E_INVAL;
  msfm_ctx* ctx = ba->ctx;
  hipStream_t s = ctx->stream;
  if (cam_pose) HIP_TRY(ctx, hipMemcpyAsync(cam_pose, ba->cam.p, sizeof(double) * 6 * (size_t)ba->Nc, hipMemcpyDeviceToHost, s));
  if (cam_model) HIP_TRY(ctx, hipMemcpyAsync(cam_model, ba->model.p, sizeof(double) * 3 * (size_t)ba->Nm, hipMemcpyDeviceToHost, s));
  if (point && ba->Np) HIP_TRY(ctx, hipMemcpyAsync(point, ba->pt.p, sizeof(double) * 3 * (size_t)ba->Np, hipMemcpyDeviceToHost, s));
  HIP_TRY(ctx, hipStreamSynchronize(s));
  return MSFM_OK;
}

const double* ba_device_points(const msfm_ba* ba) { return ba->pt.p; }

struct BaRunState {
  bool lin_pending = false;
  double lin_huber = 1.0;
  bool m_zeroed = false;
};
struct AsmHandover {
  ReduceJobs jobs;
  bool modelsum_rides = false;
  ModelSumArgs modelsum;
  AsmHandover() { jobs.count = 0; }
};

static BaPtrs make_ptrs(msfm_ba* ba, bool candidate, double huber) {
  BaPtrs P;
  P.A = ba->A; P.AE = ba->AE; P.ncb = ba->ncb; P.nmb = ba->nmb; P.npb = ba->npb; P.NCR = ba->NCR;
  P.cam = candidate ? ba->cam_c.p : ba->cam.p;
  P.rot = candidate ? ba->rot_c.p : ba->rot.p;
  P.model = candidate ? ba->model_c.p : ba->model.p;
  P.pt = candidate ? ba->pt_c.p : ba->pt.p;
  P.o_cam = ba->o_cam.p; P.o_model = ba->o_model.p; P.o_pt = ba->o_pt.p; P.o_cb = ba->o_cb.p; P.o_mb = ba->o_mb.p;
  P.o_pb = ba->o_pb.p; P.o_cpos = ba->o_cpos.p; P.o_pm = ba->o_pm.p;
  P.o_x = ba->o_x.p; P.o_y = ba->o_y.p; P.o_w = ba->o_w.p;
  P.lin_r = ba->lin_r.p; P.lin_Jc = ba->lin_Jc.p; P.lin_Jm = ba->lin_Jm.p;
  P.scale_c = ba->scale_c.p; P.scale_m = ba->scale_m.p; P.scale_p = ba->scale_p.p;
  P.huber = huber;
  return P;
}

static int allreduce(msfm_ba* ba, double* buf, size_t count, int op) {
  msfm_ctx* ctx = ba->ctx;
  if (ctx->world <= 1) return MSFM_OK;
  KTimer t(ctx, count > 4096 ? "ba_allreduce_system" : "ba_allreduce_small");
  const int rc = ctx->allreduce(ctx->allreduce_user, buf, count, op, (void*)ctx->stream);
  if (rc != 0) return msfm_set_error(ctx, MSFM_E_DEVICE, "all-reduce hook failed: %d", rc);
  return MSFM_OK;
}

static void enqueue_linearize_rest(msfm_ba* ba, BaRunState& st, bool candidate, double huber, const double* spec = nullptr) {
  msfm_ctx* ctx = ba->ctx;
  hipStream_t s = ctx->stream;
  const BaPartials& L = ba->parts;
  BaPtrs P = make_ptrs(ba, candidate, huber);
  KTimer t(ctx, "ba_linearize");
  if (L.x_frozen.n) hipLaunchKernelGGL(k_linearize<true>, dim3(L.x_frozen.n), dim3(256), 0, s, P, ba->AE, ba->partial_x.p + L.x_frozen.off, spec);
  if (L.x_gps.n) hipLaunchKernelGGL(k_gps<true>, dim3(L.x_gps.n), dim3(256), 0, s, ba->ncb, ba->cb_cam.p, P.cam, ba->gps.p, ba->gps_weight, huber, ba->scale_c.p, ba->g_r.p, ba->g_J.p, ba->partial_x.p + L.x_gps.off, spec);
  st.lin_pending = true;
  st.lin_huber = huber;
}

static void launch_point(msfm_ba* ba, const BaRunState& st, const msfm_ba_options* opt, double radius, bool reuse_diag, int mode, bool store_rows,
                         bool candidate, const double* spec) {
  msfm_ctx* ctx = ba->ctx;
  KTimer t(ctx, "ba_point");
  PointPtrs Q;
  Q.B = make_ptrs(ba, candidate, st.lin_huber);
  Q.map = ba->map; Q.npb = ba->npb; Q.NCR = std::max(1, ba->NCR); Q.pt_first = ba->pt_first.p;
  Q.pm_first = ba->pm_first.p; Q.pm_mb = ba->pm_mb.p;
  Q.diag_p = ba->diag_p.p; Q.ptL = ba->ptL.p; Q.ptg = ba->ptg.p;
  Q.T = ba->T.p; Q.Tu = ba->Tu.p; Q.Tm = ba->Tm.p; Q.Tmu = ba->Tmu.p;
  Q.radius = radius; Q.dmin = opt->min_lm_diagonal; Q.dmax = opt->max_lm_diagonal;
  Q.reuse_diag = reuse_diag; Q.mode = mode; Q.fail = ba->fail.p;
  Q.store_rows = store_rows ? 1 : 0; Q.cost_partial = ba->partial_x.p + ba->parts.x_point.off;
  const FoldTables& F = ba->fold;
  Q.fold_wg = F.on ? F.wg_fold.p : nullptr; Q.fold_wg_pass_first = F.wg_pass_first.p; Q.fold_slot_rank = F.slot_rank.p;
  Q.fold_pass = F.pass.p; Q.fold_stream = F.stream.p; Q.fold_partial = F.partial.p;
  Q.fold_mc_partial = (F.on && F.mc_on) ? F.mc_partial.p : nullptr;
  Q.spec = spec;
  hipLaunchKernelGGL(k_point, dim3(ba->nblk_pt), dim3(256), 0, ctx->stream, Q, ba->gmax_buf.p + ba->parts.g_point.off);
}

static int ba_zero_map(const msfm_ba* ba, ZeroMap& Z) {
  const int nb64 = ba->npad / 64;
  if (ba->ctx->world > 1 || nb64 > 256) return 0;
  Z.nb = nb64;
  for (int b = 0; b < nb64; b++) { Z.lev[b] = 127; Z.lo[b] = 0; Z.hi[b] = 0x7fff; }
  for (int lv = 0; lv < ba->plan.n_levels; lv++)
    for (int k = 0; k < ba->plan.level[lv].K; k++) {
      const msfm_chol_node& nd = ba->plan.level[lv].node[k];
      for (int b = nd.begin / 64; b < nd.end / 64; b++) { Z.lev[b] = (unsigned char)lv; Z.lo[b] = (short)nd.leaf_lo; Z.hi[b] = (short)nd.leaf_hi; }
    }
  return nb64 * (nb64 + 1) / 2;
}
static bool asm_beside_ok(const msfm_ba* ba) {
  const FoldTables& F = ba->fold;
  return ba->env.asm_beside && ba->ctx->world <= 1 && !ba->ctx->profile && ba->ncb > 0 && ba->nmb <= 1 && ba->n_fchunks > 0 && F.on && F.all &&
         (ba->mc.n_blocks == 0 || (F.mc_on && F.mc_all)) && ba->npad / 64 <= 256;
}
enum AsmForm { ASM_PLAIN, ASM_FUSED, ASM_BESIDE };
static AsmForm asm_form(const msfm_ba* ba) {
  if (asm_beside_ok(ba)) return ASM_BESIDE;
  if (ba->n_fchunks > 0 && (ba->fold.on || ba->cc.n_pairs < 262144)) return ASM_FUSED;
  return ASM_PLAIN;
}

static SumsArgs make_sums(msfm_ba* ba, double huber, bool beside) {
  const size_t ncr = (size_t)std::max(1, ba->NCR);
  SumsArgs a;
  a.n_zero = beside ? 0 : ba_zero_map(ba, a.Z);
  a.M = ba->M.p; a.ld = ba->npad;
  const bool mc_sparse = ba->fold.on && ba->fold.mc_on;
  a.mc_n = mc_sparse ? ba->fold.mc_n_live : ba->mc.n_chunks; a.mc_start = ba->mc.ch_start.p; a.mc_end = ba->mc.ch_end.p; a.mc_pa = ba->mc.pa.p; a.mc_pb = ba->mc.pb.p;
  a.mc_live = mc_sparse ? ba->fold.mc_live_chunk.p : nullptr; a.mc_partial = ba->mc.partial.p;
  a.mm_n = ba->mm.n_chunks; a.mm_start = ba->mm.ch_start.p; a.mm_end = ba->mm.ch_end.p; a.mm_pa = ba->mm.pa.p; a.mm_pb = ba->mm.pb.p; a.mm_partial = ba->mm.partial.p;
  a.cc_n = ba->fold.on ? ba->fold.n_live : ba->cc.n_chunks; a.cc_start = ba->cc.ch_start.p; a.cc_end = ba->cc.ch_end.p; a.cc_pa = ba->cc.pa.p; a.cc_pb = ba->cc.pb.p;
  a.cc_live = ba->fold.on ? ba->fold.live_chunk.p : nullptr; a.cc_partial = ba->cc.partial.p;
  a.T = ba->T.p; a.Tm = ba->Tm.p; a.Tmu = ba->Tmu.p; a.plane = ncr;
  a.f_n = ba->n_fchunks; a.f_start = ba->f_start.p; a.f_end = ba->f_end.p; a.P = make_ptrs(ba, false, huber);
  a.R = CamRows{ba->cm_pt.p, ba->cm_X.p, ba->cm_xyw.p, ba->cm_xyw.p + ncr, ba->cm_xyw.p + 2 * ncr, ba->chunk_cam.p};
  a.Tu = ba->Tu.p; a.cpos_pb = ba->cpos_pb.p; a.f_partial = ba->f_partial.p;
  a.n_mc_wg = cdiv(a.mc_n, 4); a.n_mm_wg = cdiv(a.mm_n, 4); a.n_cc_wg = cdiv(a.cc_n, 4); a.n_ftf_wg = cdiv(a.f_n, 4);
  memset(&a.fs, 0, sizeof a.fs);
  if (beside) {
    FoldSumArgs& f = a.fs;
    f.n_cc = ba->cc.n_blocks; f.n_mc = ba->mc.n_blocks; f.mo = ba->mo;
    f.n_cc_wg = cdiv(cdiv(f.n_cc, 3), 4); f.n_mc_wg = cdiv(f.n_mc, 4);
    f.cc_row = ba->cc.blk_row.p; f.cc_col = ba->cc.blk_col.p; f.cc_range = ba->fold.blk_range.p; f.cc_fold_partial = ba->fold.partial.p;
    f.mc_row = ba->mc.blk_row.p; f.mc_col = ba->mc.blk_col.p; f.mc_range = ba->fold.mc_range.p; f.mc_fold_partial = ba->fold.mc_partial.p;
    f.cb_off = ba->cb_off.p;
  }
  return a;
}
static AsmArgs make_asm(const msfm_ba* ba, double radius, int lead) {
  AsmArgs aa;
  aa.n_cc = ba->cc.n_blocks; aa.n_mc = ba->mc.n_blocks; aa.n_mm = ba->mm.n_blocks; aa.n_rhs = cdiv(6 * ba->ncb, 64);
  aa.cc_row = ba->cc.blk_row.p; aa.cc_col = ba->cc.blk_col.p; aa.cc_first = (ba->fold.on && ba->fold.all) ? nullptr : ba->cc.blk_chunk_first.p; aa.cc_partial = ba->cc.partial.p;
  aa.cc_fold_first = ba->fold.on ? ba->fold.blk_range.p : nullptr; aa.cc_live = ba->fold.on ? ba->fold.blk_live.p : nullptr; aa.cc_fold_partial = ba->fold.partial.p;
  aa.mc_row = ba->mc.blk_row.p; aa.mc_col = ba->mc.blk_col.p; aa.mc_partial = ba->mc.partial.p;
  const bool fmc = ba->fold.on && ba->fold.mc_on;
  aa.mc_first = (fmc && ba->fold.mc_all) ? nullptr : ba->mc.blk_chunk_first.p;
  aa.mc_fold_range = fmc ? ba->fold.mc_range.p : nullptr; aa.mc_fold_partial = ba->fold.mc_partial.p;
  aa.mm_row = ba->mm.blk_row.p; aa.mm_col = ba->mm.blk_col.p; aa.mm_first = ba->mm.blk_chunk_first.p; aa.mm_partial = ba->mm.partial.p;
  aa.cb_mb = ba->cb_mb.p; aa.cb_off = ba->cb_off.p; aa.camftf = ba->camftf.p; aa.diag_c = ba->diag_c.p; aa.modelsum = ba->modelsum.p;
  aa.diag_m = ba->diag_m.p; aa.radius = radius; aa.ncb = ba->ncb; aa.mo = ba->mo; aa.n = ba->nsys; aa.ld = ba->npad; aa.lead = lead; aa.M = ba->M.p;
  aa.n_padcol = ba->ctx->world <= 1 ? ba->n_padcol : 0;
  aa.padcol = ba->padcol.p;
  return aa;
}

static int run_assemble(msfm_ba* ba, BaRunState& st, const msfm_ba_options* opt, double radius, bool reuse_diag, int mode, bool point_enqueued = false,
                        AsmHandover* out = nullptr) {
  msfm_ctx* ctx = ba->ctx;
  hipStream_t s = ctx->stream;
  const bool will_solve = out != nullptr;
  const int ncb = ba->ncb, nmb = ba->nmb;
  const int lead = ctx->rank == 0 ? 1 : 0;
  const BaPartials& L = ba->parts;
  const bool store_rows = st.lin_pending;
  st.lin_pending = false;
  if (!point_enqueued) launch_point(ba, st, opt, radius, reuse_diag, mode, store_rows, false, nullptr);
  const AsmForm form = mode == 0 ? asm_form(ba) : ASM_PLAIN;
  const bool fused = form != ASM_PLAIN, beside = form == ASM_BESIDE;
  auto launch_pairs = [&]() {
    const size_t ncr = (size_t)std::max(1, ba->NCR);
    if (ba->mc.n_chunks)
      hipLaunchKernelGGL((k_pairs<3, 6, false>), dim3(cdiv(ba->mc.n_chunks, 4)), dim3(256), 0, s, ba->mc.n_chunks, ba->mc.ch_start.p,
                         ba->mc.ch_end.p, ba->mc.pa.p, ba->mc.pb.p, ba->Tm.p, ba->T.p, (const double*)nullptr, ncr, ba->mc.partial.p);
    if (ba->mm.n_chunks)
      hipLaunchKernelGGL((k_pairs<3, 3, true>), dim3(cdiv(ba->mm.n_chunks, 4)), dim3(256), 0, s, ba->mm.n_chunks, ba->mm.ch_start.p,
                         ba->mm.ch_end.p, ba->mm.pa.p, ba->mm.pb.p, ba->Tm.p, ba->Tm.p, ba->Tmu.p, (size_t)0, ba->mm.partial.p);
    if (ba->cc.n_chunks)
      hipLaunchKernelGGL((k_pairs<6, 6, false>), dim3(cdiv(ba->cc.n_chunks, 4)), dim3(256), 0, s, ba->cc.n_chunks, ba->cc.ch_start.p,
                         ba->cc.ch_end.p, ba->cc.pa.p, ba->cc.pb.p, ba->T.p, ba->T.p, (const double*)nullptr, ncr, ba->cc.partial.p);
  };
  const bool m_zeroed = st.m_zeroed;
  if (mode == 0) { st.m_zeroed = false; ba->asm_paths = beside ? MSFM_PATH_ASM_BESIDE : 0; }
  auto zero_system = [&]() -> int {
    ZeroMap Z;
    const int n_zero = ba_zero_map(ba, Z);
    if (n_zero) hipLaunchKernelGGL(k_zero_system, dim3(n_zero), dim3(256), 0, s, ba->M.p, ba->npad, Z);
    else HIP_TRY(ctx, hipMemsetAsync(ba->M.p, 0, sizeof(double) * (size_t)ba->npad * ba->npad, s));
    return MSFM_OK;
  };
  {
    KTimer t(ctx, "ba_ftf");
    if (fused) {
      const SumsArgs a = make_sums(ba, st.lin_huber, beside);
      if (beside ? !m_zeroed : a.n_zero == 0) MSFM_TRY(zero_system());
      hipLaunchKernelGGL(k_sums, dim3(a.n_zero + a.n_mc_wg + a.n_mm_wg + a.n_cc_wg + a.n_ftf_wg + a.fs.n_mc_wg + a.fs.n_cc_wg), dim3(256), 0, s, a);
    } else if (ba->n_fchunks) {
      const size_t ncr = (size_t)std::max(1, ba->NCR);
      const CamRows R{ba->cm_pt.p, ba->cm_X.p, ba->cm_xyw.p, ba->cm_xyw.p + ncr, ba->cm_xyw.p + 2 * ncr, ba->chunk_cam.p};
      hipLaunchKernelGGL(k_ftf, dim3(cdiv(ba->n_fchunks, 4)), dim3(256), 0, s, ba->n_fchunks, ba->f_start.p, ba->f_end.p,
                         make_ptrs(ba, false, st.lin_huber), R, ba->Tu.p, ba->cpos_pb.p, ba->f_partial.p);
    }
    if (ncb) {
      CamFinish fin;
      memset(&fin, 0, sizeof fin);
      if (beside) fin = CamFinish{ba->M.p, ba->npad, ba->nsys, ba->mo, ba->cb_off.p, ba->cb_mb.p, radius, ba->n_padcol, ba->padcol.p};
      hipLaunchKernelGGL(k_camftf, dim3(ncb + (beside ? cdiv(ba->n_padcol, 128) : 0)), dim3(128), 0, s, ncb, ba->cam_chunk_first.p, ba->f_partial.p, ba->camftf.p,
                         ba->g_r.p, ba->g_J.p, (ba->has_gps && lead) ? 1 : 0, ctx->world <= 1 ? 1 : 0, ba->diag_c.p, ba->scale_c.p,
                         reuse_diag ? 1 : 0, mode, opt->min_lm_diagonal, opt->max_lm_diagonal, ba->gmax_buf.p + L.g_cam.off, fin);
    }
  }
  if (ncb) MSFM_TRY(allreduce(ba, ba->camftf.p, (size_t)ncb * PSTRIDE, MSFM_REDUCE_SUM));
  {
    KTimer t(ctx, "ba_ftf");
    if (ncb && ctx->world > 1)
      hipLaunchKernelGGL(k_cam_post, dim3(cdiv(6 * ncb, 256)), dim3(256), 0, s, ncb, ba->camftf.p, ba->diag_c.p, ba->scale_c.p,
                         reuse_diag ? 1 : 0, mode, opt->min_lm_diagonal, opt->max_lm_diagonal, ba->gmax_buf.p + L.g_cam.off);
    if (nmb) {
      ModelFinish fin;
      memset(&fin, 0, sizeof fin);
      if (beside) fin = ModelFinish{ba->M.p, ba->npad, ba->nsys, ba->mo, ba->mm.n_blocks, ba->mm.blk_row.p, ba->mm.blk_col.p, ba->mm.blk_chunk_first.p, ba->mm.partial.p, radius};
      const ModelSumArgs ma{nmb, ba->mcam_first.p, ba->mcam.p, ba->camftf.p, ba->modelsum.p, ba->diag_m.p, ba->scale_m.p, reuse_diag ? 1 : 0, mode,
                            opt->min_lm_diagonal, opt->max_lm_diagonal, ba->gmax_buf.p + L.g_model.off, fin};
      if (beside && will_solve && ba->env.solve_riders && ba->plan.n_levels > 0 && ba->nred > 0) {
        out->modelsum_rides = true;
        out->modelsum = ma;
      } else {
        hipLaunchKernelGGL(k_modelsum, dim3(nmb), dim3(beside ? 128 : 64), 0, s, ma);
      }
    }
  }
  if (mode == 1) return MSFM_OK;
  {
    ReduceJobs rj;
    rj.count = 1;
    rj.job[0] = {ba->gmax_buf.p, L.sum_g, S_GMAX, 1};
    if (store_rows) {
      rj.job[1] = {ba->partial_x.p, L.sum_x[lead], S_XCOST, 0};
      rj.count = 2;
    }
    rj.fail = ba->fail.p;
    rj.fail_slot = S_FAIL;
    if (beside && will_solve) {
      out->jobs = rj;
    } else {
      hipLaunchKernelGGL(k_reduce, dim3(rj.count), dim3(1024), 0, s, rj, ba->swrite);
    }
  }
  if (!fused) {
    KTimer t(ctx, "ba_schur_pairs");
    launch_pairs();
  }
  {
    KTimer t(ctx, "ba_assemble");
    if (!fused) MSFM_TRY(zero_system());
    const AsmArgs aa = make_asm(ba, radius, lead);
    const int nasm = aa.n_cc + aa.n_mc + aa.n_mm + aa.n_rhs + cdiv(aa.n_padcol, 64);
    if (nasm && !beside) hipLaunchKernelGGL(k_asm_all, dim3(nasm), dim3(64), 0, s, aa);
  }
  hipError_t e = hipGetLastError();
  if (e != hipSuccess) return msfm_set_error(ctx, MSFM_E_DEVICE, "assemble launch: %s", hipGetErrorString(e));
  if (ctx->world > 1) {
    if (ba->n_ublk > 0) {
      const int nb = cdiv(ba->n_ublk * 36, 256);
      const size_t nblk = (size_t)ba->n_ublk * 36, nslab = (size_t)(ba->nsys - ba->mo + 1) * ba->npad;
      double* slab = ba->M.p + (size_t)ba->mo * ba->npad;
      hipLaunchKernelGGL(k_pack_blocks<true>, dim3(nb), dim3(256), 0, s, ba->n_ublk, ba->u_row.p, ba->u_col.p, ba->cb_off.p, ba->M.p, ba->npad, ba->pack.p);
      HIP_TRY(ctx, hipMemcpyAsync(ba->pack.p + nblk, slab, sizeof(double) * nslab, hipMemcpyDeviceToDevice, s));
      MSFM_TRY(allreduce(ba, ba->pack.p, nblk + nslab, MSFM_REDUCE_SUM));
      hipLaunchKernelGGL(k_pack_blocks<false>, dim3(nb), dim3(256), 0, s, ba->n_ublk, ba->u_row.p, ba->u_col.p, ba->cb_off.p, ba->M.p, ba->npad, ba->pack.p);
      HIP_TRY(ctx, hipMemcpyAsync(slab, ba->pack.p + nblk, sizeof(double) * nslab, hipMemcpyDeviceToDevice, s));
    } else {
      MSFM_TRY(allreduce(ba, ba->M.p, (size_t)(ba->nsys + 1) * ba->npad, MSFM_REDUCE_SUM));
    }
  }
  if (ba->n_padcol && ctx->world > 1) hipLaunchKernelGGL(k_pad_diag, dim3(cdiv(ba->n_padcol, 256)), dim3(256), 0, s, ba->n_padcol, ba->padcol.p, ba->M.p, ba->npad);
  return MSFM_OK;
}

__global__ void k_scal_pack(const double* __restrict__ sloc, double* __restrict__ scal, int rank, int world) {
  const int i = threadIdx.x;
  if (i < S_GMAX) scal[i] = sloc[i];
  if (i < world) scal[S_RANK0 + i] = i == rank ? sloc[S_GMAX] : 0.0;
}
__global__ void k_scal_unpack(double* __restrict__ scal, int world) {
  double g = 0.0;
  for (int r = 0; r < world; r++) g = fmax(g, scal[S_RANK0 + r]);
  scal[S_GMAX] = g;
}

static int reduce_scalars(msfm_ba* ba) {
  msfm_ctx* ctx = ba->ctx;
  if (ctx->world <= 1) return MSFM_OK;
  if (S_RANK0 + ctx->world > S_N) return msfm_set_error(ctx, MSFM_E_INVAL, "too many ranks for the scalar block");
  hipLaunchKernelGGL(k_scal_pack, dim3(1), dim3(64), 0, ctx->stream, ba->sloc.p, ba->scal.p, ctx->rank, ctx->world);
  MSFM_TRY(allreduce(ba, ba->scal.p, (size_t)S_RANK0 + ctx->world, MSFM_REDUCE_SUM));
  hipLaunchKernelGGL(k_scal_unpack, dim3(1), dim3(1), 0, ctx->stream, ba->scal.p, ctx->world);
  return MSFM_OK;
}

static void publish_scalars(msfm_ba* ba, const LmDecide& D) {
  msfm_ctx* ctx = ba->ctx;
  const unsigned long long seq = ++ba->scal_seq;
  hipLaunchKernelGGL(k_publish_scalars, dim3(1), dim3(64), 0, ctx->stream, ba->scal.p, ba->h_scal_dev, seq, ba->fail.p, D, ba->spec.p);
}
static int wait_scalars(msfm_ba* ba) {
  msfm_ctx* ctx = ba->ctx;
  const unsigned long long seq = ba->scal_seq;
  const double limit_s = msfm_env_process().sync_timeout_s;
  const volatile unsigned long long* flag = reinterpret_cast<const volatile unsigned long long*>(ba->h_scal + H_SEQ);
  unsigned long long spins = 0;
  const auto t0 = std::chrono::steady_clock::now();
  while (__atomic_load_n(flag, __ATOMIC_ACQUIRE) != seq) {
    if ((++spins & 0x3FFFFull) == 0) {
      const hipError_t q = hipStreamQuery(ctx->stream);
      if (q != hipSuccess && q != hipErrorNotReady) HIP_TRY(ctx, q);
      if (q == hipSuccess && __atomic_load_n(flag, __ATOMIC_ACQUIRE) != seq)
        return msfm_set_error(ctx, MSFM_E_DEVICE, "the iteration's scalars did not arrive although the stream is idle");
      if (std::chrono::duration<double>(std::chrono::steady_clock::now() - t0).count() > limit_s)
        return msfm_set_error(ctx, MSFM_E_DEVICE, "device did not finish an LM iteration within %.0f s (MSFM_SYNC_TIMEOUT_S)", limit_s);
    }
  }
  return MSFM_OK;
}

static BackPtrs make_back(msfm_ba* ba, double huber) {
  BackPtrs Q;
  Q.B = make_ptrs(ba, false, huber);
  Q.map = ba->map; Q.npb = ba->npb; Q.ncb = ba->ncb; Q.pt_first = ba->pt_first.p; Q.pb_pt = ba->pb_pt.p;
  Q.ptL = ba->ptL.p; Q.z = ba->z.p; Q.pt_c = ba->pt_c.p; Q.cm_Xc = ba->cm_Xc.p;
// ... 11 lines not shown
  a.z = ba->z.p; a.has_gps = (ba->has_gps && lead && ncb) ? 1 : 0; a.g_r = ba->g_r.p; a.g_J = ba->g_J.p; a.mcc_partial = ba->partial.p + L.m_rest[lead].off;
  a.P = make_ptrs(ba, true, opt->huber_delta);
  a.n_cost = ba->nblk_obs; a.cost_partial = ba->partial4.p + L.c_rows.off;
  a.n_gps = L.c_gps.n;
  a.cb_cam = ba->cb_cam.p; a.cam_c = a.P.cam; a.gps = ba->gps.p; a.gps_weight = ba->gps_weight; a.huber = opt->huber_delta; a.scale_c = ba->scale_c.p;
  a.g_r_w = ba->g_r.p; a.g_J_w = ba->g_J.p;
  return a;
}

static int run_solve(msfm_ba* ba, BaRunState& st, const msfm_ba_options* opt, const AsmHandover& h) {
  msfm_ctx* ctx = ba->ctx;
  hipStream_t s = ctx->stream;
  const int ncb = ba->ncb, nmb = ba->nmb, npb = ba->npb;
  const int lead = ctx->rank == 0 ? 1 : 0;
  const BaPartials& L = ba->parts;
  const double* zsolved = ba->zsys.p;
  const double wrep = lead ? 1.0 : 0.0;
  msfm_chol_riders riders;
  SolveEpilogue ep;
  ba->rider_paths = 0;
  if (ba->nred > 0) {
    double* const zcur = ba->zsys.p + (size_t)ba->zflip * (ba->npad + 8);
    double* const znext = ba->zsys.p + (size_t)(ba->zflip ^ 1) * (ba->npad + 8);
    if (h.modelsum_rides) { riders.modelsum = &h.modelsum; ba->rider_paths |= MSFM_PATH_RIDER_MODELSUM; }
    if (ba->env.solve_riders && L.u_point.n >= L.u_step.n) {
      ep = SolveEpilogue{ba->col_param.p, ba->col_slot.p, 6 * ncb, ba->scale_c.p, ba->scale_m.p, ba->cam.p, ba->model.p, ba->cam_c.p, ba->model_c.p,
                         ba->z.p, ba->upd_dx2.p, ba->upd_x2.p, ba->fail.p, wrep};
      riders.epilogue = &ep;
    }
    const int rc = msfm_chol_factor_solve(ctx, ba->env, ba->M.p, ba->npad, ba->nsys, ba->Linv.p, ba->w.p, zcur, ba->fail.p,
                                          ba->plan.n_levels > 0 ? &ba->plan : nullptr, znext, ba->chol_ws, &ba->solve_paths, &riders);
    if (rc != MSFM_OK) {
      (void)msfm_chol_fill_pending(ctx, ba->zsys.p, 2 * (ba->npad + 8));
      ba->rider_paths = 0;
      return rc;
    }
    ba->zflip ^= 1;
    zsolved = zcur;
  }
  {
    KTimer t(ctx, "ba_backsub");
    const bool in_solve = riders.epilogue_ran;
    if (in_solve) ba->rider_paths |= MSFM_PATH_RIDER_UPDATE;
    if (ba->nred > 0 && !in_solve)
      hipLaunchKernelGGL(k_update_params, dim3(L.u_step.n), dim3(256), 0, s, ncb, nmb, ba->cb_cam.p, ba->mb_model.p, ba->cb_off.p, ba->mo, zsolved,
                         ba->scale_c.p, ba->scale_m.p, ba->cam.p, ba->cam_c.p, ba->model.p, ba->model_c.p, ba->z.p, ba->fail.p,
                         ba->partial2.p + L.u_step.off, ba->partial3.p + L.u_step.off, wrep);
    if (npb) {
      const UpdateSums U{in_solve ? L.u_step.n : 0, ba->nred, ba->upd_dx2.p, ba->upd_x2.p, ba->partial2.p + L.u_step.off, ba->partial3.p + L.u_step.off};
      hipLaunchKernelGGL(k_backsub, dim3(L.u_point.n), dim3(256), 0, s, make_back(ba, st.lin_huber), ba->partial.p + L.m_point.off,
                         ba->partial2.p + L.u_point.off, ba->partial3.p + L.u_point.off, U);
    } else {
      hipLaunchKernelGGL(k_rot_cache, dim3(cdiv(std::max(1, ba->Nc), 256)), dim3(256), 0, s, ba->Nc, ba->cam_c.p, ba->rot_c.p);
    }
  }
  {
    KTimer t(ctx, "ba_cost");
    const TailArgs a = make_tail(ba, opt, lead);
    hipLaunchKernelGGL(k_tail, dim3(a.n_zero + a.n_mcc + a.n_cost + a.n_gps), dim3(256), 0, s, a);
    st.m_zeroed = a.n_zero > 0;
    ReduceJobs rj;
    rj.count = 4;
    rj.job[0] = {ba->partial.p, L.sum_m[lead], S_MCC, 0};
    rj.job[1] = {ba->partial2.p, L.sum_u, S_DX2, 0};
    rj.job[2] = {ba->partial3.p, L.sum_u, S_X2, 0};
    rj.job[3] = {ba->partial4.p, L.sum_c[lead], S_COST, 0};
    for (int j = 0; j < h.jobs.count; j++) rj.job[rj.count++] = h.jobs.job[j];
    rj.fail = ba->fail.p;
    rj.fail_slot = S_FAIL;
    hipLaunchKernelGGL(k_reduce, dim3(rj.count), dim3(1024), 0, s, rj, ba->swrite);
  }
  hipError_t e = hipGetLastError();
  if (e != hipSuccess) return msfm_set_error(ctx, MSFM_E_DEVICE, "solve launch: %s", hipGetErrorString(e));
  return MSFM_OK;
}

MSFM_API int msfm_ba_run(msfm_ba* ba, const msfm_ba_options* opt, msfm_ba_summary* sum) {
  if (!ba || !opt || !sum) return MSFM_E_INVAL;
  msfm_ctx* ctx = ba->ctx;
  if (ctx->world != ba->world_at_create)
    return msfm_set_error(ctx, MSFM_E_INVAL, "msfm_ctx_set_allreduce must be called before msfm_ba_create");
  HIP_TRY(ctx, hipSetDevice(ctx->device));
  hipStream_t s = ctx->stream;
  struct Events {
    hipEvent_t a = nullptr, b = nullptr;
    ~Events() { if (a) (void)hipEventDestroy(a); if (b) (void)hipEventDestroy(b); }
  } evs;
  hipEvent_t& ev0 = evs.a;
  hipEvent_t& ev1 = evs.b;
  const auto run_t0 = std::chrono::steady_clock::now();
  const bool verbose = msfm_env_process().verbose && ctx->rank == 0;
  auto lap = [&](const char* what) {
    if (verbose) fprintf(stderr, "msfm: run %-31s %7.2f ms\n", what, std::chrono::duration<double, std::milli>(std::chrono::steady_clock::now() - run_t0).count());
  };
  HIP_TRY(ctx, hipEventCreate(&ev0));
  HIP_TRY(ctx, hipEventCreate(&ev1));
  HIP_TRY(ctx, hipEventRecord(ev0, s));
  sum->num_residuals = ba->n_residuals;
  sum->num_reduced_params = ba->nred;
  sum->num_successful_steps = sum->num_unsuccessful_steps = 0;
  sum->setup_ms = ba->setup_ms;
  int rows = 0;
  auto push = [&](const msfm_ba_iteration& it) {
    if (sum->iterations && rows < sum->iterations_capacity) sum->iterations[rows] = it;
    rows++;
  };
  const int ncb = ba->ncb, nmb = ba->nmb, npb = ba->npb;
  if (ncb) hipLaunchKernelGGL(k_fill, dim3(cdiv(6 * ncb, 256)), dim3(256), 0, s, 6 * ncb, 1.0, ba->scale_c.p);
  if (nmb) hipLaunchKernelGGL(k_fill, dim3(cdiv(3 * nmb, 256)), dim3(256), 0, s, 3 * nmb, 1.0, ba->scale_m.p);
  if (npb) hipLaunchKernelGGL(k_fill, dim3(cdiv(3 * npb, 256)), dim3(256), 0, s, 3 * npb, 1.0, ba->scale_p.p);
  hipLaunchKernelGGL(k_rot_cache, dim3(cdiv(std::max(1, ba->Nc), 256)), dim3(256), 0, s, ba->Nc, ba->cam.p, ba->rot.p);
  {
    const size_t n0 = 6 * (size_t)ba->Nc, n1 = 3 * (size_t)ba->Nm, n2 = 3 * (size_t)ba->Np;
    hipLaunchKernelGGL(k_copy3, dim3(cdiv((long)std::max(n0, std::max(n1, n2)), 256)), dim3(256), 0, s, n0, ba->cam.p, ba->cam_c.p, n1,
                       ba->model.p, ba->model_c.p, n2, ba->pt.p, ba->pt_c.p);
  }
  if (ba->NCR > 0)
    hipLaunchKernelGGL(k_cam_points, dim3(cdiv(ba->NCR, 256)), dim3(256), 0, s, ba->NCR, ba->cm_pt.p, ba->pt.p, ba->cm_X.p, ba->cm_Xc.p);
  lap("scales reset");
  hipLaunchKernelGGL(k_zero_int, dim3(1), dim3(1), 0, s, ba->fail.p);
  BaRunState st;
  double radius = opt->initial_trust_region_radius, decrease_factor = 2.0;
  bool reuse_diag = false;
  enqueue_linearize_rest(ba, st, false, opt->huber_delta);
  lap("first evaluate enqueued");
  if (opt->jacobi_scaling) {
    MSFM_TRY(run_assemble(ba, st, opt, radius, false, 1));
    if (ncb) hipLaunchKernelGGL(k_make_scale, dim3(cdiv(6 * ncb, 256)), dim3(256), 0, s, 6 * ncb, ba->diag_c.p, ba->scale_c.p);
    if (nmb) hipLaunchKernelGGL(k_make_scale, dim3(cdiv(3 * nmb, 256)), dim3(256), 0, s, 3 * nmb, ba->diag_m.p, ba->scale_m.p);
    if (npb) hipLaunchKernelGGL(k_make_scale, dim3(cdiv(3 * npb, 256)), dim3(256), 0, s, 3 * npb, ba->diag_p.p, ba->scale_p.p);
    enqueue_linearize_rest(ba, st, false, opt->huber_delta);
  }
  int iteration = 0, num_invalid = 0, termination = 0;
  lap("iteration zero enqueued");
  double x_cost = 0.0;
  bool spec_inflight = false;
  auto assemble_and_step = [&](bool point_enqueued) -> int {
    LmDecide D;
    D.fresh = st.lin_pending ? 1 : 0;
    D.on = (iteration < opt->max_num_iterations && radius > opt->min_trust_region_radius) ? 1 : 0;
    AsmHandover h;
    MSFM_TRY(run_assemble(ba, st, opt, radius, reuse_diag, 0, point_enqueued, D.on ? &h : nullptr));
    if (D.on) MSFM_TRY(run_solve(ba, st, opt, h));
    MSFM_TRY(reduce_scalars(ba));
    D.x_cost = x_cost; D.radius = radius;
    D.min_relative_decrease = opt->min_relative_decrease; D.parameter_tolerance = opt->parameter_tolerance;
    D.function_tolerance = opt->function_tolerance; D.max_radius = opt->max_trust_region_radius; D.min_radius = opt->min_trust_region_radius;
    publish_scalars(ba, D);
    spec_inflight = false;
    if (D.on && ba->spec_on) {
      enqueue_linearize_rest(ba, st, true, opt->huber_delta, ba->spec.p);
      launch_point(ba, st, opt, radius, false, 0, true, true, ba->spec.p);
      st.lin_pending = false;
      spec_inflight = true;
    }
    MSFM_TRY(wait_scalars(ba));
    return MSFM_OK;
  };
  MSFM_TRY(assemble_and_step(false));
  x_cost = ba->h_scal[S_XCOST];
  msfm_ba_iteration it;
  memset(&it, 0, sizeof it);
  it.cost = x_cost; it.gradient_max_norm = ba->h_scal[S_GMAX]; it.trust_region_radius = radius;
  it.step_is_valid = 1; it.step_is_successful = 1;
  sum->initial_cost = x_cost;
  for (;;) {
    if (it.step_is_successful && iteration > 0) sum->num_successful_steps++;
    it.trust_region_radius = radius;
    push(it);
    if (verbose && iteration < 6) lap("iteration read back");
    if (opt->progress_to_stdout && ctx->rank == 0)
      printf("%4d  cost %.6e  change %.3e  |grad| %.3e  |step| %.3e  rho %.3e  radius %.3e\n", iteration, it.cost,
             it.cost_change, it.gradient_max_norm, it.step_norm, it.relative_decrease, radius);
    if (iteration >= opt->max_num_iterations) { termination = MSFM_BA_NO_CONVERGENCE; break; }
    if (it.gradient_max_norm <= opt->gradient_tolerance) { termination = MSFM_BA_CONVERGENCE_GRADIENT; break; }
    if (radius <= opt->min_trust_region_radius) { termination = MSFM_BA_MIN_RADIUS; break; }
    const double prev_gmax = it.gradient_max_norm;
    memset(&it, 0, sizeof it);
    iteration++;
    if ((long)ba->h_scal[S_FAIL] >= MSFM_FAIL_SYNC)
      return msfm_set_error(ctx, MSFM_E_DEVICE, "a bounded in-kernel wait of the back substitution ran out (MSFM_SYNC_TIMEOUT_S)");
    const int code = (int)ba->h_scal[H_CODE];
    const double mcc = ba->h_scal[S_MCC], cand_cost = ba->h_scal[S_COST], dx2 = ba->h_scal[S_DX2], x2 = ba->h_scal[S_X2];
    if (code < LM_INVALID || code > LM_REJECT) return msfm_set_error(ctx, MSFM_E_DEVICE, "no verdict for the step (code %d)", code);
    it.step_is_valid = code != LM_INVALID;
    bool relinearise = false;
    if (!it.step_is_valid) {
      if (++num_invalid >= opt->max_num_consecutive_invalid_steps) { termination = MSFM_BA_FAILURE; break; }
      radius = radius / decrease_factor; decrease_factor *= 2.0; reuse_diag = true;
      it.cost = x_cost; it.gradient_max_norm = prev_gmax;
      sum->num_unsuccessful_steps++;
    } else {
      num_invalid = 0;
      it.step_norm = std::sqrt(dx2);
      (void)x2;
      if (code == LM_PARAM_TOL) { termination = MSFM_BA_CONVERGENCE_PARAMETER; break; }
      it.cost_change = x_cost - cand_cost;
      if (code == LM_FUNC_TOL) { termination = MSFM_BA_CONVERGENCE_FUNCTION; break; }
      it.relative_decrease = (x_cost - cand_cost) / mcc;
      if (code == LM_ACCEPT) {
        ba->cam.swap(ba->cam_c); ba->model.swap(ba->model_c); ba->pt.swap(ba->pt_c); ba->rot.swap(ba->rot_c); ba->cm_X.swap(ba->cm_Xc);
        relinearise = true;
        it.step_is_successful = 1;
        radius = ba->h_scal[H_RADIUS];
        decrease_factor = 2.0; reuse_diag = false;
      } else {
        it.step_is_successful = 0; it.cost = cand_cost; it.gradient_max_norm = prev_gmax;
        radius = radius / decrease_factor; decrease_factor *= 2.0; reuse_diag = true;
        sum->num_unsuccessful_steps++;
      }
    }
    bool point_enqueued = false;
    if (relinearise) {
      if (spec_inflight && radius > opt->min_trust_region_radius) {
        st.lin_pending = true;
        st.lin_huber = opt->huber_delta;
        point_enqueued = true;
      } else {
        enqueue_linearize_rest(ba, st, false, opt->huber_delta);
      }
    }
    MSFM_TRY(assemble_and_step(point_enqueued));
    if (relinearise) {
      x_cost = ba->h_scal[S_XCOST];
      it.cost = x_cost;
      it.gradient_max_norm = ba->h_scal[S_GMAX];
    }
  }
  sum->termination = termination;
  sum->num_iterations = rows - 1;
  sum->final_cost = x_cost;
  lap("loop done");
  HIP_TRY(ctx, hipEventRecord(ev1, s));
  HIP_TRY(ctx, hipEventSynchronize(ev1));
  lap("synchronised");
// ... 16 lines not shown
```

### metricsfm_amd/csrc/common.h

```cpp
#pragma once
#include <hip/hip_runtime.h>

#include <cstdarg>
#include <cstdint>
#include <cstdio>
#include <cstring>
#include <algorithm>
#include <cstdlib>
#include <initializer_list>
#include <string>
#include <thread>
#include <utility>
#include <vector>

#include "../../include/msfm.h"
#include "chol_plan.h"

#define MSFM_API extern "C" __attribute__((visibility("default")))

struct msfm_env {
  int chol_domains = -1;
  bool chol_launches = false;
  bool chain_force = false;
  bool chain_trace = false;
  bool create_host = false;
  long fold_min = 262144;
  bool no_fold = false;
  long lanes4_min = -1;
  bool asm_beside = true;
  bool spec = true;
  bool solve_riders = true;
  size_t pool_bytes = (size_t)16384 << 20;
  bool pool_debug = false;
  int host_threads = 0;
  double sync_timeout_s = 120.0;
  int device_share = 1;
  bool verbose = false;
  int multi_fail_rank = -1;
  int localize_lds_max = 4096;
};
msfm_env msfm_env_read();
const msfm_env& msfm_env_process();

struct msfm_ctx {
  int device = 0;
  hipStream_t stream = nullptr;
  std::string err;
  msfm_allreduce_fn allreduce = nullptr;
  void* allreduce_user = nullptr;
  int rank = 0, world = 1;
  int device_share = 1;
  bool profile = false;
  struct Stat { std::string name; uint64_t launches = 0; double ms = 0; };
  std::vector<Stat> stats;
  struct Pending { int stat; hipEvent_t a, b; };
  std::vector<Pending> pending;
  std::vector<hipEvent_t> event_pool;
  void* ba_scratch = nullptr;
  void (*ba_scratch_free)(void*) = nullptr;
  int children = 0;
  bool orphaned = false;
  void* rccl_lib = nullptr;
  void* rccl_comm = nullptr;
  void* rccl_allreduce = nullptr;
  void* rccl_comm_destroy = nullptr;
  void* rccl_error_string = nullptr;
};
void msfm_ctx_child_released(msfm_ctx* ctx);

int msfm_set_error(msfm_ctx* ctx, int code, const char* fmt, ...);

#define HIP_TRY(ctx, expr)                                                                      \
  do {                                                                                          \
    hipError_t e_ = (expr);                                                                     \
    if (e_ != hipSuccess)                                                                       \
      return msfm_set_error((ctx), MSFM_E_DEVICE, "%s:%d %s -> %s", __FILE__, __LINE__, #expr,  \
                            hipGetErrorString(e_));                                             \
  } while (0)

#define MSFM_TRY(expr)            \
  do {                            \
    int rc_ = (expr);             \
    if (rc_ != MSFM_OK) return rc_; \
  } while (0)

struct KTimer {
  msfm_ctx* ctx;
  int idx = -1;
  int count = 1;
  hipEvent_t a = nullptr, b = nullptr;
  KTimer(msfm_ctx* c, const char* name);
  void stop();
  ~KTimer();
};

int msfm_stream_wait_bounded(msfm_ctx* ctx, hipStream_t s, const char* what);
void msfm_ctx_forget_rccl(msfm_ctx* ctx);
hipError_t msfm_pool_alloc(void** p, size_t bytes, size_t* capacity);
void msfm_pool_free(void* p, size_t capacity);
void msfm_pool_trim(int device);

template <typename T>
struct DevBuf {
  T* p = nullptr;
  size_t n = 0;
  size_t cap = 0;
  DevBuf() = default;
  DevBuf(const DevBuf&) = delete;
  DevBuf& operator=(const DevBuf&) = delete;
  ~DevBuf() { release(); }
  void swap(DevBuf& o) {
    std::swap(p, o.p); std::swap(n, o.n); std::swap(cap, o.cap);
  }
  void release() {
// ... 399 lines not shown
```

### metricsfm_amd/csrc/ctx.hip

```cpp
#include "common.h"

int msfm_set_error(msfm_ctx* ctx, int code, const char* fmt, ...) {
  char buf[512];
  va_list ap;
  va_start(ap, fmt);
  vsnprintf(buf, sizeof buf, fmt, ap);
  va_end(ap);
  if (ctx) ctx->err = buf;
  return code;
}

msfm_env msfm_env_read() {
  msfm_env E;
  auto get = [](const char* name) { return getenv(name); };
  auto num = [&](const char* name, int unset) { const char* e = get(name); return e ? atoi(e) : unset; };
  E.chol_domains = num("MSFM_CHOL_DOMAINS", E.chol_domains);
  E.chol_launches = get("MSFM_CHOL_LAUNCHES") != nullptr;
  E.chain_force = get("MSFM_CHAIN_FORCE") != nullptr;
  E.chain_trace = get("MSFM_CHAIN_TRACE") != nullptr;
  E.create_host = num("MSFM_CREATE_HOST", 0) != 0;
  if (const char* e = get("MSFM_FOLD_MIN")) E.fold_min = atol(e);
  E.no_fold = get("MSFM_NO_FOLD") != nullptr;
  if (const char* e = get("MSFM_LANES4_MIN")) E.lanes4_min = atol(e);
  E.asm_beside = num("MSFM_ASM_BESIDE", 1) != 0;
  E.spec = num("MSFM_SPEC", 1) != 0;
  E.solve_riders = num("MSFM_SOLVE_RIDERS", 1) != 0;
  if (const char* e = get("MSFM_POOL_MB")) E.pool_bytes = (size_t)atol(e) << 20;
  E.pool_debug = get("MSFM_POOL_DEBUG") != nullptr;
  E.host_threads = std::max(1, std::min(num("MSFM_HOST_THREADS", std::min(8, (int)std::thread::hardware_concurrency())), 64));
  if (const char* e = get("MSFM_SYNC_TIMEOUT_S")) E.sync_timeout_s = atof(e) > 0 ? atof(e) : 120.0;
  E.device_share = std::max(1, num("MSFM_DEVICE_SHARE", 1));
  E.verbose = get("MSFM_VERBOSE") != nullptr;
  E.multi_fail_rank = num("MSFM_MULTI_FAIL_RANK", -1);
  E.localize_lds_max = num("MSFM_LOCALIZE_LDS_MAX", E.localize_lds_max);
  return E;
}

const msfm_env& msfm_env_process() {
  static const msfm_env E = msfm_env_read();
  return E;
}

MSFM_API int msfm_version(void) { return MSFM_VERSION; }

MSFM_API int msfm_ctx_create(int device, msfm_ctx** out) {
  if (!out) return MSFM_E_INVAL;
  *out = nullptr;
  int n = 0;
  if (hipGetDeviceCount(&n) != hipSuccess || n <= 0) return MSFM_E_DEVICE;
  msfm_ctx* ctx = new msfm_ctx();
  if (device < 0) {
    if (hipGetDevice(&device) != hipSuccess) device = 0;
  }
  if (device >= n || hipSetDevice(device) != hipSuccess ||
      hipStreamCreateWithFlags(&ctx->stream, hipStreamNonBlocking) != hipSuccess) {
    delete ctx;
    return MSFM_E_DEVICE;
  }
  ctx->device = device;
  ctx->device_share = msfm_env_process().device_share;
  *out = ctx;
  return MSFM_OK;
}

#include <map>
#include <mutex>
namespace {
struct Pool {
  std::mutex mu;
  struct Live { size_t capacity; int device; };
  std::map<void*, Live> live;
  std::multimap<std::pair<int, size_t>, void*> free_blocks;
  size_t cached_bytes = 0;
  size_t mismatches = 0;
  size_t limit() { return msfm_env_process().pool_bytes; }
  bool debug() { return msfm_env_process().pool_debug; }
};
Pool& pool() { static Pool* p = new Pool(); return *p; }
size_t round_capacity(size_t bytes) {
  if (bytes <= 4096) return 4096;
  if (bytes <= ((size_t)2 << 20)) { size_t c = 4096; while (c < bytes) c <<= 1; return c; }
  return (bytes + ((size_t)2 << 20) - 1) & ~(((size_t)2 << 20) - 1);
}
}

hipError_t msfm_pool_alloc(void** p, size_t bytes, size_t* capacity) {
  int dev = 0;
  (void)hipGetDevice(&dev);
  const size_t want = round_capacity(bytes);
  Pool& P = pool();
  {
    std::lock_guard<std::mutex> g(P.mu);
    auto it = P.free_blocks.lower_bound({dev, want});
    if (it != P.free_blocks.end() && it->first.first == dev && it->first.second <= 2 * want) {
      *p = it->second;
      *capacity = it->first.second;
      P.cached_bytes -= it->first.second;
      P.free_blocks.erase(it);
      if (P.live.count(*p)) { fprintf(stderr, "msfm pool: block %p handed out twice\n", *p); abort(); }
      P.live[*p] = Pool::Live{*capacity, dev};
      return hipSuccess;
    }
  }
  hipError_t e = hipMalloc(p, want);
  if (e != hipSuccess) {
    msfm_pool_trim(dev);
    (void)hipGetLastError();
    e = hipMalloc(p, want);
  }
// ... 296 lines not shown
```

Baseline: 1323 iterations/s.

## Add lean run path: gradient-only final assemble, fused start kernels, cached events

On the final iteration, when no further step will be solved, the point kernel now runs a gradient-only variant that skips Schur/fold work, and run_assemble returns early without building the reduced system. The run-start fills, rotation cache, copies and camera-point gathers are merged into one kernel, the three scale builds into another, and the run events are kept on the BA object instead of being recreated per run. These target fixed per-run overhead and the wasted last linearization, at the cost of an extra kernel instantiation and a new env-controlled code path.

```diff
diff --git a/include/msfm.h b/include/msfm.h
--- a/include/msfm.h
+++ b/include/msfm.h
@@ -171,7 +171,9 @@
   int assemble_paths;
   int rider_paths;
   long long fold_parts, fold_crit_steps, fold_crit_steps_unsplit, fold_wave_steps;
+  int run_paths;
 } msfm_ba_layout;
+#define MSFM_PATH_RUN_GRAD_LAST (1 << 16)
 #define MSFM_PATH_ASM_BESIDE 1
 #define MSFM_PATH_RIDER_MODELSUM (1 << 8)
 #define MSFM_PATH_RIDER_UPDATE (1 << 9)
diff --git a/metricsfm_amd/_abi.py b/metricsfm_amd/_abi.py
--- a/metricsfm_amd/_abi.py
+++ b/metricsfm_amd/_abi.py
@@ -18,6 +18,7 @@
 MSFM_PATH_ASM_BESIDE = 1
 MSFM_PATH_RIDER_MODELSUM = 1 << 8
 MSFM_PATH_RIDER_UPDATE = 1 << 9
+PATH_RUN_GRAD_LAST = 1 << 16
 
 
 def MSFM_PATH_LEVEL_CHAIN(level):
@@ -44,7 +45,7 @@
                 ("mc_entries", C.c_longlong), ("mc_entries_folded", C.c_longlong), ("fold_mc_slots", C.c_int), ("solve_paths", C.c_int),
                 ("npb_S", C.c_int), ("npb_L", C.c_int), ("npb_X", C.c_int), ("npb_S4", C.c_int), ("assemble_paths", C.c_int),
                 ("rider_paths", C.c_int), ("fold_parts", C.c_longlong), ("fold_crit_steps", C.c_longlong),
-                ("fold_crit_steps_unsplit", C.c_longlong), ("fold_wave_steps", C.c_longlong)]
+                ("fold_crit_steps_unsplit", C.c_longlong), ("fold_wave_steps", C.c_longlong), ("run_paths", C.c_int)]
 
 
 class FransacOptions(C.Structure):
diff --git a/metricsfm_amd/capi.py b/metricsfm_amd/capi.py
--- a/metricsfm_amd/capi.py
+++ b/metricsfm_amd/capi.py
@@ -1205,7 +1205,7 @@
                               mc_entries=lay.mc_entries, mc_entries_folded=lay.mc_entries_folded, mc_slots=lay.fold_mc_slots,
                               parts=lay.fold_parts, crit_steps=lay.fold_crit_steps, crit_steps_unsplit=lay.fold_crit_steps_unsplit,
                               wave_steps=lay.fold_wave_steps),
-                    solve_paths=lay.solve_paths, assemble_paths=lay.assemble_paths, rider_paths=lay.rider_paths, npb_S=lay.npb_S, npb_L=lay.npb_L, npb_X=lay.npb_X, npb_S4=lay.npb_S4)
+                    solve_paths=lay.solve_paths, assemble_paths=lay.assemble_paths, rider_paths=lay.rider_paths, run_paths=lay.run_paths, npb_S=lay.npb_S, npb_L=lay.npb_L, npb_X=lay.npb_X, npb_S4=lay.npb_S4)
 
     def upload(self, cam_pose=None, cam_model=None, point=None):
         cp, cm, pt = A.as_c(cam_pose, np.float64), A.as_c(cam_model, np.float64), A.as_c(point, np.float64)
diff --git a/metricsfm_amd/csrc/ba.hip b/metricsfm_amd/csrc/ba.hip
--- a/metricsfm_amd/csrc/ba.hip
+++ b/metricsfm_amd/csrc/ba.hip
@@ -243,14 +243,16 @@
 #define FOLD_WORDS 1024
 #define FOLD_PASS_SLOTS 128
 #define FOLD_PASS_QUADS 256
-template <int LPP>
+enum { PT_FULL = 0, PT_GRAD = 1 };
+template <int LPP, int FORM>
 __device__ __forceinline__ void k_point_body(const PointPtrs& P, double* __restrict__ gmax_partial, double* sh, double* park, unsigned* ent_s) {
   constexpr int GW = LPP ? LPP : 8;
   constexpr bool single = LPP != 0;
+  constexpr bool grad_only = FORM == PT_GRAD;
   const int tid = threadIdx.x, sub = tid & (GW - 1);
   const int pb = ptmap_wg_first(P.map, blockIdx.x) + tid / GW;
   const bool act = pb < ptmap_wg_end(P.map, blockIdx.x);
-  const bool fold = single && P.fold_wg != nullptr && P.mode != 1 && P.fold_wg[blockIdx.x] != 0;
+  const bool fold = !grad_only && single && P.fold_wg != nullptr && P.mode != 1 && P.fold_wg[blockIdx.x] != 0;
   const int wv = __builtin_amdgcn_readfirstlane(tid >> 6);
   auto stage = [&](int off, int words) {
     if (256 * wv < words)
@@ -270,7 +272,7 @@
   auto lin_row = [&](int i) {
     double r0, r1, jcs[12], jms[6], jps[6];
     const double ci = obs_linearize(P.B, i, r0, r1, jcs, jms, jps);
-    if constexpr (single) {
+    if constexpr (single && !grad_only) {
 #pragma unroll
       for (int k = 0; k < 12; k++) park[k * 256 + tid] = jcs[k];
 #pragma unroll
@@ -293,7 +295,12 @@
 
   double gmax = 0.0;
   double l00 = 1, l10 = 0, l11 = 1, l20 = 0, l21 = 0, l22 = 1, i00 = 1, i11 = 1, i22 = 1, u0 = 0, u1 = 0, u2 = 0;
-  if (act) {
+  if constexpr (grad_only) {
+    if (act && sub == 0) {
+      const double* sp = P.B.scale_p + 3 * (size_t)pb;
+      gmax = fmax(fabs(g0 / sp[0]), fmax(fabs(g1 / sp[1]), fabs(g2 / sp[2])));
+    }
+  } else if (act) {
     double* dg = P.diag_p + 3 * (size_t)pb;
     if (P.mode == 1) {
       if (sub == 0) { dg[0] = V00; dg[1] = V11; dg[2] = V22; }
@@ -331,7 +338,7 @@
       }
     }
   }
-  if (P.mode != 1) {
+  if (!grad_only && P.mode != 1) {
     const int wl = tid & 63, tsrc = GW == 16 ? ((wl & 3) << 4) | (wl >> 2) : GW == 4 ? ((wl & 15) << 2) | (wl >> 4) : ((wl & 7) << 3) | (wl >> 3);
     const bool need_T = !fold || P.fold_mc_partial == nullptr;
     auto round = [&](int rd, double (&Tk)[18], int& cpk) {
@@ -584,16 +591,17 @@
   const double t = block_max256(gmax, sh);
   if (threadIdx.x == 0) gmax_partial[blockIdx.x] = t;
 }
+template <int FORM>
 __global__ __launch_bounds__(256) __attribute__((amdgpu_waves_per_eu(3, 3))) void k_point(PointPtrs P, double* __restrict__ gmax_partial) {
   __shared__ double sh[4];
-  __shared__ double park[24 * 256];
-  __shared__ __attribute__((aligned(16))) unsigned ent_s[FOLD_WORDS];
+  __shared__ double park[FORM == PT_GRAD ? 1 : 24 * 256];
+  __shared__ __attribute__((aligned(16))) unsigned ent_s[FORM == PT_GRAD ? 4 : FOLD_WORDS];
   if (P.spec && P.spec[0] == 0.0) return;
   const int lanes = ptmap_lanes(P.map, blockIdx.x);
-  if (lanes == 4) k_point_body<4>(P, gmax_partial, sh, park, ent_s);
-  else if (lanes == 8) k_point_body<8>(P, gmax_partial, sh, park, ent_s);
-  else if (lanes == 16) k_point_body<16>(P, gmax_partial, sh, park, ent_s);
-  else k_point_body<0>(P, gmax_partial, sh, park, ent_s);
+  if (lanes == 4) k_point_body<4, FORM>(P, gmax_partial, sh, park, ent_s);
+  else if (lanes == 8) k_point_body<8, FORM>(P, gmax_partial, sh, park, ent_s);
+  else if (lanes == 16) k_point_body<16, FORM>(P, gmax_partial, sh, park, ent_s);
+  else k_point_body<0, FORM>(P, gmax_partial, sh, park, ent_s);
 }
 
 __global__ __launch_bounds__(256) void k_cam_rows(int A, const int* __restrict__ o_cpos, const int* __restrict__ o_pt, const double* __restrict__ o_x,
@@ -829,6 +837,14 @@
 __global__ void k_make_scale(int n, const double* __restrict__ norm2, double* __restrict__ scale) {
   const int i = blockIdx.x * blockDim.x + threadIdx.x;
   if (i < n) scale[i] = 1.0 / (1.0 + sqrt(norm2[i]));
+}
+__global__ __launch_bounds__(256) void k_make_scale3(int n0, const double* __restrict__ norm0, double* __restrict__ scale0, int n1,
+                                                     const double* __restrict__ norm1, double* __restrict__ scale1, int n2,
+                                                     const double* __restrict__ norm2, double* __restrict__ scale2) {
+  const int i = blockIdx.x * 256 + threadIdx.x;
+  if (i < n0) scale0[i] = 1.0 / (1.0 + sqrt(norm0[i]));
+  if (i < n1) scale1[i] = 1.0 / (1.0 + sqrt(norm1[i]));
+  if (i < n2) scale2[i] = 1.0 / (1.0 + sqrt(norm2[i]));
 }
 
 template <int DA, int DB, bool WITH_U, bool SPARSE = false>
@@ -1486,6 +1502,44 @@
 __global__ void k_fill(int n, double v, double* __restrict__ p) {
   const int i = blockIdx.x * 256 + threadIdx.x;
   if (i < n) p[i] = v;
+}
+struct RunStartArgs {
+  int b_fill, b_rot, b_copy, b_pts;
+  int n_sc, n_sm, n_sp; double *scale_c, *scale_m, *scale_p; int* fail;
+  int Nc; const double* cam; double* rot;
+  size_t n0, n1, n2; const double *a0, *a1, *a2; double *b0, *b1, *b2;
+  int ncr; const int* cm_pt; const double* pt; double *X0, *X1;
+};
+__global__ __launch_bounds__(256) void k_run_start(RunStartArgs a) {
+  int b = blockIdx.x;
+  if (b < a.b_fill) {
+    const int i = b * 256 + threadIdx.x;
+    if (i < a.n_sc) a.scale_c[i] = 1.0;
+    if (i < a.n_sm) a.scale_m[i] = 1.0;
+    if (i < a.n_sp) a.scale_p[i] = 1.0;
+    if (i == 0) *a.fail = 0;
+    return;
+  }
+  b -= a.b_fill;
+  if (b < a.b_rot) {
+    const int c = b * 256 + threadIdx.x;
+    if (c < a.Nc) msfm_rot_prepare(a.cam + 6 * (size_t)c, a.rot + 4 * (size_t)c);
+    return;
+  }
+  b -= a.b_rot;
+  if (b < a.b_copy) {
+    const size_t i = (size_t)b * 256 + threadIdx.x;
+    if (i < a.n0) a.b0[i] = a.a0[i];
+    if (i < a.n1) a.b1[i] = a.a1[i];
+    if (i < a.n2) a.b2[i] = a.a2[i];
+    return;
+  }
+  b -= a.b_copy;
+  const int e = b * 256 + threadIdx.x;
+  if (e >= a.ncr) return;
+  const size_t p = (size_t)a.cm_pt[e];
+#pragma unroll
+  for (int j = 0; j < 3; j++) { const double v = a.pt[3 * p + j]; a.X0[3 * (size_t)e + j] = v; a.X1[3 * (size_t)e + j] = v; }
 }
 
 template <bool PACK>
@@ -1584,9 +1638,11 @@
   DevBuf<double> pack;
   int zflip = 0;
   unsigned long long scal_seq = 0;
+  hipEvent_t ev_run[2] = {nullptr, nullptr};
   int solve_paths = 0;
   int asm_paths = 0;
   int rider_paths = 0;
+  int run_paths = 0;
 };
 
 struct CamGraph {
@@ -2007,6 +2063,7 @@
   ba->chol_ws = nullptr;
   if (ba->h_scal) (void)hipHostFree(ba->h_scal);
   if (ba->h_fail) (void)hipHostFree(ba->h_fail);
+  for (hipEvent_t e : ba->ev_run) if (e) (void)hipEventDestroy(e);
   delete ba;
   msfm_ctx_child_released(ctx);
 }
@@ -3628,6 +3685,7 @@
   out->solve_paths = ba->solve_paths;
   out->assemble_paths = ba->asm_paths;
   out->rider_paths = ba->rider_paths;
+  out->run_paths = ba->run_paths;
   out->npb_S = ba->map.nQ + ba->map.nS; out->npb_L = ba->map.nL; out->npb_X = ba->map.nX; out->npb_S4 = ba->n_short4;
   return MSFM_OK;
 }
@@ -3706,7 +3764,7 @@
 }
 
 static void launch_point(msfm_ba* ba, const BaRunState& st, const msfm_ba_options* opt, double radius, bool reuse_diag, int mode, bool store_rows,
-                         bool candidate, const double* spec) {
+                         bool candidate, const double* spec, bool grad_only = false) {
   msfm_ctx* ctx = ba->ctx;
   KTimer t(ctx, "ba_point");
   PointPtrs Q;
@@ -3723,7 +3781,9 @@
   Q.fold_pass = F.pass.p; Q.fold_stream = F.stream.p; Q.fold_partial = F.partial.p;
   Q.fold_mc_partial = (F.on && F.mc_on) ? F.mc_partial.p : nullptr;
   Q.spec = spec;
-  hipLaunchKernelGGL(k_point, dim3(ba->nblk_pt), dim3(256), 0, ctx->stream, Q, ba->gmax_buf.p + ba->parts.g_point.off);
+  double* const gmax_partial = ba->gmax_buf.p + ba->parts.g_point.off;
+  if (grad_only) hipLaunchKernelGGL(k_point<PT_GRAD>, dim3(ba->nblk_pt), dim3(256), 0, ctx->stream, Q, gmax_partial);
+  else hipLaunchKernelGGL(k_point<PT_FULL>, dim3(ba->nblk_pt), dim3(256), 0, ctx->stream, Q, gmax_partial);
 }
 
 static int ba_zero_map(const msfm_ba* ba, ZeroMap& Z) {
@@ -3795,7 +3855,7 @@
 }
 
 static int run_assemble(msfm_ba* ba, BaRunState& st, const msfm_ba_options* opt, double radius, bool reuse_diag, int mode, bool point_enqueued = false,
-                        AsmHandover* out = nullptr) {
+                        AsmHandover* out = nullptr, bool grad_only = false) {
   msfm_ctx* ctx = ba->ctx;
   hipStream_t s = ctx->stream;
   const bool will_solve = out != nullptr;
@@ -3804,9 +3864,10 @@
   const BaPartials& L = ba->parts;
   const bool store_rows = st.lin_pending;
   st.lin_pending = false;
-  if (!point_enqueued) launch_point(ba, st, opt, radius, reuse_diag, mode, store_rows, false, nullptr);
+  if (!point_enqueued) launch_point(ba, st, opt, radius, reuse_diag, mode, store_rows, false, nullptr, grad_only);
   const AsmForm form = mode == 0 ? asm_form(ba) : ASM_PLAIN;
-  const bool fused = form != ASM_PLAIN, beside = form == ASM_BESIDE;
+  const bool fused = form != ASM_PLAIN && !grad_only, beside = form == ASM_BESIDE && !grad_only;
+  const bool keep_diag = reuse_diag || grad_only;
   auto launch_pairs = [&]() {
     const size_t ncr = (size_t)std::max(1, ba->NCR);
     if (ba->mc.n_chunks)
@@ -3820,7 +3881,7 @@
                          ba->cc.ch_end.p, ba->cc.pa.p, ba->cc.pb.p, ba->T.p, ba->T.p, (const double*)nullptr, ncr, ba->cc.partial.p);
   };
   const bool m_zeroed = st.m_zeroed;
-  if (mode == 0) { st.m_zeroed = false; ba->asm_paths = beside ? MSFM_PATH_ASM_BESIDE : 0; }
+  if (mode == 0) { st.m_zeroed = false; ba->asm_paths = form == ASM_BESIDE ? MSFM_PATH_ASM_BESIDE : 0; }
   auto zero_system = [&]() -> int {
     ZeroMap Z;
     const int n_zero = ba_zero_map(ba, Z);
@@ -3846,7 +3907,7 @@
       if (beside) fin = CamFinish{ba->M.p, ba->npad, ba->nsys, ba->mo, ba->cb_off.p, ba->cb_mb.p, radius, ba->n_padcol, ba->padcol.p};
       hipLaunchKernelGGL(k_camftf, dim3(ncb + (beside ? cdiv(ba->n_padcol, 128) : 0)), dim3(128), 0, s, ncb, ba->cam_chunk_first.p, ba->f_partial.p, ba->camftf.p,
                          ba->g_r.p, ba->g_J.p, (ba->has_gps && lead) ? 1 : 0, ctx->world <= 1 ? 1 : 0, ba->diag_c.p, ba->scale_c.p,
-                         reuse_diag ? 1 : 0, mode, opt->min_lm_diagonal, opt->max_lm_diagonal, ba->gmax_buf.p + L.g_cam.off, fin);
+                         keep_diag ? 1 : 0, mode, opt->min_lm_diagonal, opt->max_lm_diagonal, ba->gmax_buf.p + L.g_cam.off, fin);
     }
   }
   if (ncb) MSFM_TRY(allreduce(ba, ba->camftf.p, (size_t)ncb * PSTRIDE, MSFM_REDUCE_SUM));
@@ -3854,12 +3915,12 @@
     KTimer t(ctx, "ba_ftf");
     if (ncb && ctx->world > 1)
       hipLaunchKernelGGL(k_cam_post, dim3(cdiv(6 * ncb, 256)), dim3(256), 0, s, ncb, ba->camftf.p, ba->diag_c.p, ba->scale_c.p,
-                         reuse_diag ? 1 : 0, mode, opt->min_lm_diagonal, opt->max_lm_diagonal, ba->gmax_buf.p + L.g_cam.off);
+                         keep_diag ? 1 : 0, mode, opt->min_lm_diagonal, opt->max_lm_diagonal, ba->gmax_buf.p + L.g_cam.off);
     if (nmb) {
       ModelFinish fin;
       memset(&fin, 0, sizeof fin);
       if (beside) fin = ModelFinish{ba->M.p, ba->npad, ba->nsys, ba->mo, ba->mm.n_blocks, ba->mm.blk_row.p, ba->mm.blk_col.p, ba->mm.blk_chunk_first.p, ba->mm.partial.p, radius};
-      const ModelSumArgs ma{nmb, ba->mcam_first.p, ba->mcam.p, ba->camftf.p, ba->modelsum.p, ba->diag_m.p, ba->scale_m.p, reuse_diag ? 1 : 0, mode,
+      const ModelSumArgs ma{nmb, ba->mcam_first.p, ba->mcam.p, ba->camftf.p, ba->modelsum.p, ba->diag_m.p, ba->scale_m.p, keep_diag ? 1 : 0, mode,
                             opt->min_lm_diagonal, opt->max_lm_diagonal, ba->gmax_buf.p + L.g_model.off, fin};
       if (beside && will_solve && ba->env.solve_riders && ba->plan.n_levels > 0 && ba->nred > 0) {
         out->modelsum_rides = true;
@@ -3885,6 +3946,11 @@
     } else {
       hipLaunchKernelGGL(k_reduce, dim3(rj.count), dim3(1024), 0, s, rj, ba->swrite);
     }
+  }
+  if (grad_only) {
+    hipError_t e = hipGetLastError();
+    if (e != hipSuccess) return msfm_set_error(ctx, MSFM_E_DEVICE, "assemble launch: %s", hipGetErrorString(e));
+    return MSFM_OK;
   }
   if (!fused) {
     KTimer t(ctx, "ba_schur_pairs");
@@ -4062,19 +4128,15 @@
     return msfm_set_error(ctx, MSFM_E_INVAL, "msfm_ctx_set_allreduce must be called before msfm_ba_create");
   HIP_TRY(ctx, hipSetDevice(ctx->device));
   hipStream_t s = ctx->stream;
-  struct Events {
-    hipEvent_t a = nullptr, b = nullptr;
-    ~Events() { if (a) (void)hipEventDestroy(a); if (b) (void)hipEventDestroy(b); }
-  } evs;
-  hipEvent_t& ev0 = evs.a;
-  hipEvent_t& ev1 = evs.b;
+  hipEvent_t& ev0 = ba->ev_run[0];
+  hipEvent_t& ev1 = ba->ev_run[1];
   const auto run_t0 = std::chrono::steady_clock::now();
   const bool verbose = msfm_env_process().verbose && ctx->rank == 0;
   auto lap = [&](const char* what) {
     if (verbose) fprintf(stderr, "msfm: run %-31s %7.2f ms\n", what, std::chrono::duration<double, std::milli>(std::chrono::steady_clock::now() - run_t0).count());
   };
-  HIP_TRY(ctx, hipEventCreate(&ev0));
-  HIP_TRY(ctx, hipEventCreate(&ev1));
+  if (!ev0) HIP_TRY(ctx, hipEventCreate(&ev0));
+  if (!ev1) HIP_TRY(ctx, hipEventCreate(&ev1));
   HIP_TRY(ctx, hipEventRecord(ev0, s));
   sum->num_residuals = ba->n_residuals;
   sum->num_reduced_params = ba->nred;
@@ -4086,19 +4148,30 @@
     rows++;
   };
   const int ncb = ba->ncb, nmb = ba->nmb, npb = ba->npb;
-  if (ncb) hipLaunchKernelGGL(k_fill, dim3(cdiv(6 * ncb, 256)), dim3(256), 0, s, 6 * ncb, 1.0, ba->scale_c.p);
-  if (nmb) hipLaunchKernelGGL(k_fill, dim3(cdiv(3 * nmb, 256)), dim3(256), 0, s, 3 * nmb, 1.0, ba->scale_m.p);
-  if (npb) hipLaunchKernelGGL(k_fill, dim3(cdiv(3 * npb, 256)), dim3(256), 0, s, 3 * npb, 1.0, ba->scale_p.p);
-  hipLaunchKernelGGL(k_rot_cache, dim3(cdiv(std::max(1, ba->Nc), 256)), dim3(256), 0, s, ba->Nc, ba->cam.p, ba->rot.p);
-  {
-    const size_t n0 = 6 * (size_t)ba->Nc, n1 = 3 * (size_t)ba->Nm, n2 = 3 * (size_t)ba->Np;
+  const bool lean = ba->env.run_lean;
+  const size_t n0 = 6 * (size_t)ba->Nc, n1 = 3 * (size_t)ba->Nm, n2 = 3 * (size_t)ba->Np;
+  if (lean) {
+    RunStartArgs a;
+    a.n_sc = 6 * ncb; a.n_sm = 3 * nmb; a.n_sp = 3 * npb; a.scale_c = ba->scale_c.p; a.scale_m = ba->scale_m.p; a.scale_p = ba->scale_p.p; a.fail = ba->fail.p;
+    a.Nc = ba->Nc; a.cam = ba->cam.p; a.rot = ba->rot.p;
+    a.n0 = n0; a.n1 = n1; a.n2 = n2; a.a0 = ba->cam.p; a.a1 = ba->model.p; a.a2 = ba->pt.p; a.b0 = ba->cam_c.p; a.b1 = ba->model_c.p; a.b2 = ba->pt_c.p;
+    a.ncr = ba->NCR; a.cm_pt = ba->cm_pt.p; a.pt = ba->pt.p; a.X0 = ba->cm_X.p; a.X1 = ba->cm_Xc.p;
+    a.b_fill = cdiv(std::max(1, std::max(a.n_sc, std::max(a.n_sm, a.n_sp))), 256);
+    a.b_rot = cdiv(ba->Nc, 256); a.b_copy = cdiv((long)std::max(n0, std::max(n1, n2)), 256); a.b_pts = cdiv(ba->NCR, 256);
+    hipLaunchKernelGGL(k_run_start, dim3(a.b_fill + a.b_rot + a.b_copy + a.b_pts), dim3(256), 0, s, a);
+    lap("run start enqueued");
+  } else {
+    if (ncb) hipLaunchKernelGGL(k_fill, dim3(cdiv(6 * ncb, 256)), dim3(256), 0, s, 6 * ncb, 1.0, ba->scale_c.p);
+    if (nmb) hipLaunchKernelGGL(k_fill, dim3(cdiv(3 * nmb, 256)), dim3(256), 0, s, 3 * nmb, 1.0, ba->scale_m.p);
+    if (npb) hipLaunchKernelGGL(k_fill, dim3(cdiv(3 * npb, 256)), dim3(256), 0, s, 3 * npb, 1.0, ba->scale_p.p);
+    hipLaunchKernelGGL(k_rot_cache, dim3(cdiv(std::max(1, ba->Nc), 256)), dim3(256), 0, s, ba->Nc, ba->cam.p, ba->rot.p);
     hipLaunchKernelGGL(k_copy3, dim3(cdiv((long)std::max(n0, std::max(n1, n2)), 256)), dim3(256), 0, s, n0, ba->cam.p, ba->cam_c.p, n1,
                        ba->model.p, ba->model_c.p, n2, ba->pt.p, ba->pt_c.p);
-  }
-  if (ba->NCR > 0)
-    hipLaunchKernelGGL(k_cam_points, dim3(cdiv(ba->NCR, 256)), dim3(256), 0, s, ba->NCR, ba->cm_pt.p, ba->pt.p, ba->cm_X.p, ba->cm_Xc.p);
-  lap("scales reset");
-  hipLaunchKernelGGL(k_zero_int, dim3(1), dim3(1), 0, s, ba->fail.p);
+    if (ba->NCR > 0)
+      hipLaunchKernelGGL(k_cam_points, dim3(cdiv(ba->NCR, 256)), dim3(256), 0, s, ba->NCR, ba->cm_pt.p, ba->pt.p, ba->cm_X.p, ba->cm_Xc.p);
+    lap("scales reset");
+    hipLaunchKernelGGL(k_zero_int, dim3(1), dim3(1), 0, s, ba->fail.p);
+  }
   BaRunState st;
   double radius = opt->initial_trust_region_radius, decrease_factor = 2.0;
   bool reuse_diag = false;
@@ -4106,21 +4179,30 @@
   lap("first evaluate enqueued");
   if (opt->jacobi_scaling) {
     MSFM_TRY(run_assemble(ba, st, opt, radius, false, 1));
-    if (ncb) hipLaunchKernelGGL(k_make_scale, dim3(cdiv(6 * ncb, 256)), dim3(256), 0, s, 6 * ncb, ba->diag_c.p, ba->scale_c.p);
-    if (nmb) hipLaunchKernelGGL(k_make_scale, dim3(cdiv(3 * nmb, 256)), dim3(256), 0, s, 3 * nmb, ba->diag_m.p, ba->scale_m.p);
-    if (npb) hipLaunchKernelGGL(k_make_scale, dim3(cdiv(3 * npb, 256)), dim3(256), 0, s, 3 * npb, ba->diag_p.p, ba->scale_p.p);
+    if (lean) {
+      const int nmax = std::max(6 * ncb, std::max(3 * nmb, 3 * npb));
+      if (nmax) hipLaunchKernelGGL(k_make_scale3, dim3(cdiv(nmax, 256)), dim3(256), 0, s, 6 * ncb, ba->diag_c.p, ba->scale_c.p, 3 * nmb, ba->diag_m.p,
+                                   ba->scale_m.p, 3 * npb, ba->diag_p.p, ba->scale_p.p);
+    } else {
+      if (ncb) hipLaunchKernelGGL(k_make_scale, dim3(cdiv(6 * ncb, 256)), dim3(256), 0, s, 6 * ncb, ba->diag_c.p, ba->scale_c.p);
+      if (nmb) hipLaunchKernelGGL(k_make_scale, dim3(cdiv(3 * nmb, 256)), dim3(256), 0, s, 3 * nmb, ba->diag_m.p, ba->scale_m.p);
+      if (npb) hipLaunchKernelGGL(k_make_scale, dim3(cdiv(3 * npb, 256)), dim3(256), 0, s, 3 * npb, ba->diag_p.p, ba->scale_p.p);
+    }
     enqueue_linearize_rest(ba, st, false, opt->huber_delta);
   }
   int iteration = 0, num_invalid = 0, termination = 0;
   lap("iteration zero enqueued");
+  ba->run_paths = 0;
   double x_cost = 0.0;
   bool spec_inflight = false;
   auto assemble_and_step = [&](bool point_enqueued) -> int {
     LmDecide D;
     D.fresh = st.lin_pending ? 1 : 0;
     D.on = (iteration < opt->max_num_iterations && radius > opt->min_trust_region_radius) ? 1 : 0;
+    const bool grad_only = lean && st.lin_pending && iteration >= opt->max_num_iterations;
     AsmHandover h;
-    MSFM_TRY(run_assemble(ba, st, opt, radius, reuse_diag, 0, point_enqueued, D.on ? &h : nullptr));
+    MSFM_TRY(run_assemble(ba, st, opt, radius, reuse_diag, 0, point_enqueued, D.on ? &h : nullptr, grad_only));
+    if (grad_only) ba->run_paths |= MSFM_PATH_RUN_GRAD_LAST;
     if (D.on) MSFM_TRY(run_solve(ba, st, opt, h));
     MSFM_TRY(reduce_scalars(ba));
     D.x_cost = x_cost; D.radius = radius;
@@ -4130,7 +4212,7 @@
     spec_inflight = false;
     if (D.on && ba->spec_on) {
       enqueue_linearize_rest(ba, st, true, opt->huber_delta, ba->spec.p);
-      launch_point(ba, st, opt, radius, false, 0, true, true, ba->spec.p);
+      launch_point(ba, st, opt, radius, false, 0, true, true, ba->spec.p, lean && iteration + 1 >= opt->max_num_iterations);
       st.lin_pending = false;
       spec_inflight = true;
     }
diff --git a/metricsfm_amd/csrc/common.h b/metricsfm_amd/csrc/common.h
--- a/metricsfm_amd/csrc/common.h
+++ b/metricsfm_amd/csrc/common.h
@@ -30,6 +30,7 @@
   bool asm_beside = true;
   bool spec = true;
   bool solve_riders = true;
+  bool run_lean = true;
   size_t pool_bytes = (size_t)16384 << 20;
   bool pool_debug = false;
   int host_threads = 0;
diff --git a/metricsfm_amd/csrc/ctx.hip b/metricsfm_amd/csrc/ctx.hip
--- a/metricsfm_amd/csrc/ctx.hip
+++ b/metricsfm_amd/csrc/ctx.hip
@@ -25,6 +25,7 @@
   E.asm_beside = num("MSFM_ASM_BESIDE", 1) != 0;
   E.spec = num("MSFM_SPEC", 1) != 0;
   E.solve_riders = num("MSFM_SOLVE_RIDERS", 1) != 0;
+  E.run_lean = num("MSFM_RUN_LEAN", 1) != 0;
   if (const char* e = get("MSFM_POOL_MB")) E.pool_bytes = (size_t)atol(e) << 20;
   E.pool_debug = get("MSFM_POOL_DEBUG") != nullptr;
   E.host_threads = std::max(1, std::min(num("MSFM_HOST_THREADS", std::min(8, (int)std::thread::hardware_concurrency())), 64));
```

Result: no change. 1327 iterations/s, median of 6 (+0.3%).
